# PNP-team/ZPrize23-gpu-submission

Hardware: AMD Instinct MI355X
Metric: gen_proof wall-clock (s), HEIGHT=15 Poseidon tree, 1/2/4/8 MI355X + HBM GB/s (lower is better)
Workload: dtype u64

## Files before the change

include/pnp_plonk.h:

```cpp
#ifndef PNP_PLONK_H
#define PNP_PLONK_H

#include <stdint.h>
#include <stddef.h>

#ifdef __cplusplus
extern "C" {
#endif


typedef struct {
    uint64_t a_eval[4];
    uint64_t b_eval[4];
    uint64_t c_eval[4];
    uint64_t d_eval[4];
} WireEvaluationsC;

typedef struct {
    uint64_t left_sigma_eval[4];
    uint64_t right_sigma_eval[4];
    uint64_t out_sigma_eval[4];
    uint64_t permutation_eval[4];
} PermutationEvaluationsC;

// ... 194 lines not shown
#define PNP_EX_TAG_STATUS    0x57A7A500ULL
#define PNP_EX_TAG_DEVICE    0xDE71CE00ULL
typedef int (*pnp_alltoall_fn)(void *user, uint64_t bytes_per_peer);
typedef int (*pnp_alltoallv_fn)(void *user, const uint64_t *send_bytes, const uint64_t *recv_bytes);
int pnp_ctx_stream(pnp_ctx *ctx, void **stream);
int pnp_set_exchange_ordered(pnp_ctx *ctx, int ordered);
int pnp_set_msm_shard(pnp_ctx *ctx, int rank, int world, pnp_allgather_fn allgather,
                      void *user, uint64_t *d_xbuf, uint64_t xbuf_bytes);
int pnp_set_exchange_a2a(pnp_ctx *ctx, pnp_alltoall_fn alltoall, void *user, uint64_t *d_a2a,
                         uint64_t a2a_bytes);
int pnp_set_exchange_v(pnp_ctx *ctx, pnp_alltoallv_fn alltoallv, void *user, uint64_t *d_send,
                       uint64_t *d_recv, uint64_t capacity_bytes);


int pnp_sync(pnp_ctx *ctx);

int pnp_ntt(pnp_ctx *ctx, uint64_t *d_inout, uint32_t lg_n, int inverse, int coset);

int pnp_coset_lde8(pnp_ctx *ctx, const uint64_t *d_coeffs, uint64_t *d_out8, uint32_t lg_n);

int pnp_commit(pnp_ctx *ctx, const uint64_t *d_points, const uint64_t *d_scalars,
               uint64_t n, CommitmentC *out);

int pnp_commit_ck(pnp_ctx *ctx, const uint64_t *d_scalars, uint64_t n, CommitmentC *out);

int pnp_commit_evals(pnp_ctx *ctx, const uint64_t *d_evals, uint64_t n, CommitmentC *out);

int pnp_hbm_usage(pnp_ctx *ctx, uint64_t out[6]);

int pnp_commit_segments(pnp_ctx *ctx, const uint64_t *d_points, uint64_t n_points, int B,
                        const uint64_t *seg_off, const uint64_t *const *d_scalars, uint64_t n,
                        CommitmentC *out);

int pnp_wire_sigma(pnp_ctx *ctx, const uint32_t *const d_var[4], uint64_t n_gates, uint64_t n_vars,
                   uint32_t lg_n, uint32_t *d_next, uint64_t *const d_sigma[4]);

int pnp_gather_witness(pnp_ctx *ctx, const uint32_t *const d_var[4], uint64_t n_gates,
                       const uint64_t *d_values, uint64_t n_vars, uint32_t lg_n, uint64_t *const d_w[4]);

int pnp_poly_eval(pnp_ctx *ctx, const uint64_t *d_coeffs, uint64_t n,
                  const uint64_t x[4], uint64_t out[4]);

int pnp_poly_div_linear(pnp_ctx *ctx, uint64_t *d_poly, uint64_t n, const uint64_t z[4]);

int pnp_prefix_product(pnp_ctx *ctx, uint64_t *d_inout, uint64_t n);

int pnp_batch_inverse(pnp_ctx *ctx, uint64_t *d_inout, uint64_t n);


int pnp_synth_random_fr(pnp_ctx *ctx, uint64_t *d_out, uint64_t n, uint64_t seed);
int pnp_synth_srs(pnp_ctx *ctx, uint64_t *d_out, uint64_t n, const uint64_t tau[4]);
int pnp_synth_circuit(pnp_ctx *ctx, uint64_t *const w[4], uint64_t *const sel[9],
                      uint64_t *const sigma[4], uint64_t n, uint64_t n_gates, uint64_t pi_pos,
                      const uint64_t pi_canon[4]);
int pnp_synth_merkle(pnp_ctx *ctx, uint32_t height, const uint64_t *consts, const uint64_t *d_leaves,
                     const uint64_t *d_blind, uint64_t *d_nodes, uint64_t *const w[4], uint64_t *const sel[9],
                     uint64_t *const sigma[4], uint64_t n, uint64_t root_canon[4]);
int pnp_synth_coset_consts(pnp_ctx *ctx, uint64_t *d_vh, uint64_t *d_x, uint32_t lg_n);

#ifdef __cplusplus
}
#endif

#ifdef __cplusplus
static_assert(sizeof(CommitmentC) == 96, "CommitmentC layout (lib.rs:231-235)");
static_assert(sizeof(ProofEvaluationsC) == 26 * 32, "ProofEvaluationsC layout");
// ... 13 lines not shown
```

zprize23-gpu-submission_amd/csrc/abi.cpp:

```cpp
#include <algorithm>
#include <dlfcn.h>
#include <array>
#include <atomic>
#include <chrono>
#include <mutex>
#include <set>
#include <thread>
#include <stdarg.h>
#include <stdlib.h>
#include <string.h>
#include "context.h"
#include "ec.cuh"
#include "protocol.h"

namespace pnp {

static thread_local char g_err[512] = "";

void set_error(const char *fmt, ...) {
    va_list ap;
    va_start(ap, fmt);
    vsnprintf(g_err, sizeof g_err, fmt, ap);
    va_end(ap);
}
// ... 767 lines not shown
}

int pnp_commit_segments(pnp_ctx *ctx, const uint64_t *d_points, uint64_t n_points, int B, const uint64_t *seg_off,
                        const uint64_t *const *d_scalars, uint64_t n, CommitmentC *out) {
    if (!ctx || !out || !seg_off || !d_scalars || B < 1 || B > 16 || (n_points && !d_points)) return PNP_E_ARG;
    for (int b = 0; b < B; b++) {
        if ((n && !d_scalars[b]) || seg_off[b] > n_points || n > n_points - seg_off[b]) {
            set_error("commit segments: MSM %d covers points [%llu, %llu) of %llu", b,
                      (unsigned long long)seg_off[b], (unsigned long long)(seg_off[b] + n),
                      (unsigned long long)n_points);
            return PNP_E_ARG;
        }
    }
    if (ctx->msm.world > 1) {
        set_error("commit segments: single-GPU operator");
        return PNP_E_ARG;
    }
    PNP_TRY({
        std::vector<uint64_t> xyzz((size_t)B * 24), aff((size_t)B * 12);
        if (n != 0) {
            DevBuf tab;
            msm_build_table(tab, d_points, n_points, msm_fold_c(n, ctx->msm.fold_c), ctx->stream);
            MsmSegs segs;
            segs.n_table = n_points;
            for (int b = 0; b < B; b++) segs.off[b] = seg_off[b];
            segs.c = msm_fold_c(n, ctx->msm.fold_c);
            msm_run_batch(ctx->msm, nullptr, d_scalars, B, n, xyzz.data(), ctx->stream, tab.u64(), false, &segs);
        }
        xyzz_to_affine_batch_host(xyzz.data(), B, aff.data());
        for (int b = 0; b < B; b++) {
            memcpy(out[b].x, &aff[12 * b], 48);
            memcpy(out[b].y, &aff[12 * b + 6], 48);
        }
    });
}

int pnp_poly_eval(pnp_ctx *ctx, const uint64_t *d, uint64_t n, const uint64_t x[4], uint64_t out[4]) {
    if (!ctx || !d || !x || !out) return PNP_E_ARG;
    PNP_TRY({
        Fr r;
        k_poly_eval(d, n, from_u64_limbs<FrP>(x), ctx->scratch_a, &r, ctx->stream);
        to_u64_limbs(r, out);
    });
}

int pnp_poly_div_linear(pnp_ctx *ctx, uint64_t *d, uint64_t n, const uint64_t z[4]) {
    if (!ctx || !d || !z) return PNP_E_ARG;
    PNP_TRY(k_poly_div_linear(d, n, from_u64_limbs<FrP>(z), ctx->scratch_a, ctx->stream));
}

int pnp_prefix_product(pnp_ctx *ctx, uint64_t *d, uint64_t n) {
    if (!ctx || !d) return PNP_E_ARG;
    PNP_TRY(k_prefix_product(d, n, ctx->scratch_a, ctx->stream));
}

int pnp_batch_inverse(pnp_ctx *ctx, uint64_t *d, uint64_t n) {
    if (!ctx || !d) return PNP_E_ARG;
    PNP_TRY(k_batch_inverse(d, n, ctx->scratch_a, ctx->stream));
}

int pnp_synth_random_fr(pnp_ctx *ctx, uint64_t *d, uint64_t n, uint64_t seed) {
    if (!ctx || !d) return PNP_E_ARG;
    PNP_TRY(k_random_fr(d, n, seed, ctx->stream));
}

int pnp_synth_srs(pnp_ctx *ctx, uint64_t *d, uint64_t n, const uint64_t tau[4]) {
// ... 615 lines not shown
                if (p && !pnp::k_any_nonzero(p, 4 * D, ctx->scratch_b, ctx->stream)) p = nullptr;
                if (p && kPkKinds[f] == kTable) {
                    pnp::DevBuf &t = tabc[f - kTableField[0]];
                    t.alloc(32 * D);
                    PNP_HIP(hipMemcpyAsync(t.p, p, 32 * D, hipMemcpyDeviceToDevice, ctx->stream));
                    pnp::ntt_run(ctx->ntt, t.u64(), lg, true, false, ctx->stream);
                    p = t.u64();
                }
                if (!p) {
                    memset(vk->polys[k].x, 0, 48);
                    memcpy(vk->polys[k].y, one, 48);
                    continue;
                }
                sc.push_back(p);
                oc.push_back(&vk->polys[k]);
            }
            for (size_t b = 0; b < sc.size(); b += 8)
                pnp::commit_affine_batch(ctx, sc.data() + b, (int)std::min<size_t>(8, sc.size() - b), D, oc.data() + b);
            lap(t_vk);
        }
        ctx->stages.push_back({"pre_upload", t_up});
        ctx->stages.push_back({"pre_permutation", t_perm});
        ctx->stages.push_back({"pre_intt", t_intt});
        ctx->stages.push_back({"pre_derive", t_derive});
        ctx->stages.push_back({"pre_vk", t_vk});
        ctx->stages.push_back({"pre_h2d_bytes", h2d_bytes});
    });
}

}

namespace {

void adopt_ck(pnp_ctx *ctx, pnp::DevBuf &up, uint64_t n_points) {
    const bool same = ctx->ck_owned.p && ctx->ck_dev == ctx->ck_owned.u64() && ctx->ck_points == n_points &&
                      !pnp::k_any_diff(up.u64(), ctx->ck_owned.u64(), 12 * n_points, ctx->scratch_b, ctx->stream);
    PNP_HIP(hipStreamSynchronize(ctx->stream));
    if (!same) {
        std::swap(ctx->ck_owned, up);
        ctx->ck_dev = ctx->ck_owned.u64();
        pnp::ck_derived_reset(ctx);
    }
    ctx->ck_points = n_points;
    ctx->ck_loaded = true;
    ctx->hbm_checked = false;
}

}

extern "C" {

int pnp_load_commit_key(pnp_ctx *ctx, const CommitKeyC *ck, uint64_t n_points, int device_ptrs) {
    if (!ctx || !ck || !ck->powers_of_g || n_points == 0) return PNP_E_ARG;
    PNP_TRY({
        tables_wait(ctx);
        PNP_HIP(hipSetDevice(ctx->device));
        ctx->ck_loaded = false;
        if (device_ptrs) {
            uint64_t h[2];
            pnp::k_hash_words(ck->powers_of_g, 12 * n_points, ctx->scratch_b, ctx->stream, h);
            const bool same = ctx->ck_hash_valid && !ctx->ck_owned.p && ctx->ck_dev == ck->powers_of_g &&
                              ctx->ck_points == n_points && h[0] == ctx->ck_hash[0] && h[1] == ctx->ck_hash[1];
            ctx->ck_owned.release();
            ctx->ck_dev = ck->powers_of_g;
            ctx->ck_points = n_points;
            if (!same) pnp::ck_derived_reset(ctx);
            ctx->ck_hash[0] = h[0];
            ctx->ck_hash[1] = h[1];
            ctx->ck_hash_valid = true;
            ctx->ck_loaded = true;
            ctx->hbm_checked = false;
        } else {
            ctx->ck_hash_valid = false;
            pnp::DevBuf up(n_points * 96);
            h2d_batch(ctx, {{up.p, ck->powers_of_g, n_points * 96}});
            adopt_ck(ctx, up, n_points);
        }
    });
}

int pnp_load_commit_key_strided(pnp_ctx *ctx, const void *points, uint64_t n_points,
                                const pnp_affine_layout *layout, int device_ptrs) {
    if (!ctx || !points || !layout || n_points == 0) return PNP_E_ARG;
    const pnp_affine_layout L = *layout;
    if (L.stride % 8 || L.x_off % 8 || L.y_off % 8 || L.x_off + 48 > L.stride || L.y_off + 48 > L.stride ||
        L.inf_off >= L.stride || (L.x_off < L.y_off + 48 && L.y_off < L.x_off + 48) ||
        (L.inf_off >= L.x_off && L.inf_off < L.x_off + 48) || (L.inf_off >= L.y_off && L.inf_off < L.y_off + 48)) {
        pnp::set_error("affine layout: stride %llu, x at %llu, y at %llu, infinity at %llu is not a G1Affine layout",
                       (unsigned long long)L.stride, (unsigned long long)L.x_off, (unsigned long long)L.y_off,
                       (unsigned long long)L.inf_off);
        return PNP_E_ARG;
    }
    PNP_TRY({
        tables_wait(ctx);
        PNP_HIP(hipSetDevice(ctx->device));
        ctx->ck_loaded = false;
        pnp::DevBuf raw;
        const uint8_t *src = static_cast<const uint8_t *>(points);
        if (!device_ptrs) {
// ... 544 lines not shown
```

zprize23-gpu-submission_amd/csrc/context.h:

```cpp
#pragma once
#include "pnp_internal.h"
#include <array>
#include <atomic>
#include <memory>
#include <thread>

struct pnp_ctx {
    int device = 0;
    hipStream_t stream = nullptr;
    hipStream_t stream_lo = nullptr;
    hipEvent_t ev_fork = nullptr, ev_w8 = nullptr, ev_z8 = nullptr;
    hipStream_t side_stream();
    pnp::NttTables ntt;
    pnp::MsmWork msm;
    pnp::DevBuf scratch_a, scratch_b;
    static constexpr int kStgThreads = 6;
    void *stg_buf[2 * kStgThreads] = {};
    hipStream_t stg_st[kStgThreads] = {};
    hipEvent_t stg_ev[2 * kStgThreads] = {};

    bool pk_loaded = false;
    uint64_t pk_n = 0;
    std::vector<pnp::DevBuf> pk_owned;
    ProverKeyC pk_dev{};
    bool pk_qm_zero = false, pk_qlookup_zero = false;
    bool pk_custom_nz[4] = {};
    pnp::DevBuf pk_sigma_n[4];
    pnp::DevBuf pk_tmp[4];
    std::map<std::string, pnp::DevBuf> pk_blk;
    int pk_mb0 = 0, pk_nb = 8, pk_blk_rank = 0, pk_blk_world = 1;
    bool pk_std_coset = false;
    pnp::DevBuf pk_pinv;
    uint64_t pk_pinv_pos = ~0ULL;
    const uint64_t *blk(const char *name) const {
        auto it = pk_blk.find(name);
        return it == pk_blk.end() ? nullptr : it->second.u64();
    }
    std::map<std::string, pnp::DevBuf> pk_blk29;
    bool pk_q29 = false;
    const uint64_t *blk29(const char *name) const {
        auto it = pk_blk29.find(name);
        return it == pk_blk29.end() ? nullptr : it->second.u64();
    }
    bool wm_loaded = false;
    uint64_t wm_gates = 0, wm_vars = 0;
    pnp::DevBuf wm_var;
    pnp::DevBuf wm_qlk;
    void wire_map_drop() {
        wm_loaded = false;
        wm_gates = wm_vars = 0;
        wm_var.release();
        wm_qlk.release();
    }
    bool ck_loaded = false;
    uint64_t ck_points = 0;
    pnp::DevBuf ck_owned;
    const uint64_t *ck_dev = nullptr;
    uint64_t ck_hash[2] = {0, 0};
    bool ck_hash_valid = false;
    pnp::DevBuf ck_table;
    uint64_t ck_table_n = 0, ck_table_p0 = 0, ck_table_p1 = 0;
    pnp::DevBuf lag_points, lag_table;
    uint64_t lag_n = 0, lag_table_n = 0, lag_table_p0 = 0, lag_table_p1 = 0;
    bool lag_ok = false;
    struct WireBases {
        bool built = false, ok = false, wires_ok = false, z_ok = false;
        bool sliced = false;
        int c = 0;
        uint64_t n = 0, total = 0, m = 0, len = 0;
        uint64_t g[5] = {}, off[5] = {};
        bool ident[5] = {};
        pnp::DevBuf grp[5], rep[5];
        pnp::DevBuf scal[5];
        pnp::DevBuf table;
        pnp::DevBuf sigma;
        pnp::DevBuf flag;
        uint64_t pk_gen = 0;
    } wb;
    uint64_t pk_gen = 0;
    std::atomic<bool> hbm_lag_off{false}, hbm_groups_off{false};
    bool hbm_checked = false;
    int defer_tables = -1;
    bool defer_now = false;
    bool tables_wanted = false;
    uint64_t proofs_started = 0;
    std::thread bg;
    std::atomic<int> bg_state{0};
    std::atomic<bool> bg_cancel{false};
    hipStream_t bg_stream = nullptr;

// ... 59 lines not shown
```

zprize23-gpu-submission_amd/csrc/msm.hip:

```cpp
#include <algorithm>
#include "msm_internal.h"
#include "ec.cuh"
#include "ec29.cuh"

namespace pnp {

constexpr uint32_t KEY_ZERO = 0xFFFFFFFFu;
template <int C, class E>
__device__ __forceinline__ void digits_of(const Fr &s, int c_rt, int W_rt, int top_sh, E emit) {
    const int c = C > 0 ? C : c_rt;
    const int W = C > 0 ? (255 + C) / C : W_rt;
    const uint32_t NB = 1u << (c - 1);
    uint32_t carry = 0;
    auto digit = [&](int w) {
        const int bit = w * c;
        const int li = bit >> 5, sh = bit & 31;
        uint32_t lo32 = 0, hi32 = 0;
#pragma unroll
        for (int k = 0; k < 8; k++) {
            lo32 = li == k ? s.v[k] : lo32;
            hi32 = li + 1 == k ? s.v[k] : hi32;
        }
        const uint64_t word = lo32 | ((uint64_t)hi32 << 32);
        uint32_t raw = (uint32_t)(word >> sh) & ((1u << c) - 1);
// ... 28 lines not shown
        digits_of<20>(s, c, W, top_sh, emit);
    else
        digits_of<0>(s, c, W, top_sh, emit);
}
__global__ void k_digits(const uint64_t *scalars, uint64_t n, int c, int W, int top_sh, uint32_t *keys) {
    uint64_t i = blockIdx.x * (uint64_t)blockDim.x + threadIdx.x;
    if (i >= n) return;
    scalar_digits(scalars, i, n, c, W, top_sh, keys, [](uint32_t) {});
}

constexpr int MSM_BATCH_MAX = 16;
struct KeyRows {
    uint64_t n;
    int vstride, off, rows;
    uint32_t id_row0;
    uint64_t id_mul;
    uint64_t id_base = 0;
    int nseg = 0;
    uint64_t seg_off[MSM_BATCH_MAX] = {};
};

#ifndef PNP_SORT_CB
#define PNP_SORT_CB 9
#endif
constexpr int SORT_CB = PNP_SORT_CB;
constexpr int SORT_FB_MAX = 11;
static_assert(SORT_CB >= 1 && SORT_CB <= 12, "PNP_SORT_CB out of range (LDS budget of k_coarse_scatter)");
__device__ __forceinline__ uint64_t cidx(int v, int nv, uint32_t b, int NBc, int wmaj, int ch, int nch) {
    if (wmaj <= 1) return ((uint64_t)v * NBc + b) * nch + ch;
    const uint32_t nbl = (uint32_t)NBc / wmaj;
    return (((uint64_t)(b / nbl) * nv + v) * nbl + b % nbl) * nch + ch;
}

__global__ __launch_bounds__(1024) void k_coarse_hist(const uint32_t *keys, KeyRows kr, int fb,
                                                      int NBc, uint64_t chunk, int nch,
                                                      uint32_t *counts, int wmaj = 1) {
    __shared__ uint32_t hist[1 << SORT_CB];
    const int v = blockIdx.y, ch = blockIdx.x;
    for (int b = threadIdx.x; b < NBc; b += blockDim.x) hist[b] = 0;
    __syncthreads();
    const uint64_t n = kr.n;
    uint64_t lo = (uint64_t)ch * chunk, hi = lo + chunk < n ? lo + chunk : n;
    const uint32_t *kb = keys + ((uint64_t)v * kr.vstride + kr.off) * n;
    const bool vec = ((n | chunk) & 3) == 0;
    for (int r = 0; r < kr.rows; r++) {
        const uint32_t *k = kb + (uint64_t)r * n;
        if (vec) {
            for (uint64_t i = lo + 4 * threadIdx.x; i < hi; i += 4 * blockDim.x) {
                uint4 q = *reinterpret_cast<const uint4 *>(k + i);
                uint32_t w[4] = {q.x, q.y, q.z, q.w};
#pragma unroll
                for (int j = 0; j < 4; j++)
                    if (w[j] != KEY_ZERO) atomicAdd(&hist[(w[j] & 0x7FFFFFFFu) >> fb], 1u);
            }
        } else {
            for (uint64_t i = lo + threadIdx.x; i < hi; i += blockDim.x) {
                uint32_t key = k[i];
                if (key != KEY_ZERO) atomicAdd(&hist[(key & 0x7FFFFFFFu) >> fb], 1u);
            }
        }
    }
    __syncthreads();
    for (int b = threadIdx.x; b < NBc; b += blockDim.x) counts[cidx(v, gridDim.y, b, NBc, wmaj, ch, nch)] = hist[b];
}

struct ScalarPtrs {
    static constexpr int MAX = MSM_BATCH_MAX;
    const uint64_t *p[MAX];
};
__global__ __launch_bounds__(1024) void k_digits_hist(ScalarPtrs sp, uint64_t n, int c, int W, int top_sh, int fb,
                                                      int NBc,
                                                      uint64_t chunk, int nch, uint32_t *keys, uint32_t *counts,
                                                      int wmaj = 1) {
    __shared__ uint32_t hist[1 << SORT_CB];
    const int v = blockIdx.y, ch = blockIdx.x;
    for (int b = threadIdx.x; b < NBc; b += blockDim.x) hist[b] = 0;
    __syncthreads();
    const uint64_t lo = (uint64_t)ch * chunk, hi = lo + chunk < n ? lo + chunk : n;
    uint32_t *kv = keys + (uint64_t)v * W * n;
    for (uint64_t i = lo + threadIdx.x; i < hi; i += blockDim.x)
        scalar_digits(sp.p[v], i, n, c, W, top_sh, kv, [&](uint32_t key) {
            if (key != KEY_ZERO) atomicAdd(&hist[(key & 0x7FFFFFFFu) >> fb], 1u);
        });
    __syncthreads();
    for (int b = threadIdx.x; b < NBc; b += blockDim.x) counts[cidx(v, gridDim.y, b, NBc, wmaj, ch, nch)] = hist[b];
}

__global__ __launch_bounds__(256) void k_scan_tiles(uint32_t *d, uint64_t n, uint32_t *tile_sums) {
    __shared__ uint32_t wsum[4];
    uint64_t base = (uint64_t)blockIdx.x * 1024;
    uint32_t v[4], loc = 0;
    for (int k = 0; k < 4; k++) {
        uint64_t i = base + threadIdx.x * 4 + k;
        v[k] = i < n ? d[i] : 0;
        loc += v[k];
    }
    uint32_t x = loc;
    int lane = threadIdx.x & 63, wv = threadIdx.x >> 6;
    for (int off = 1; off < 64; off <<= 1) {
        uint32_t y = __shfl_up(x, off, 64);
        if (lane >= off) x += y;
    }
    if (lane == 63) wsum[wv] = x;
    __syncthreads();
    uint32_t wpre = 0;
    for (int j = 0; j < wv; j++) wpre += wsum[j];
    uint32_t excl = wpre + x - loc;
    for (int k = 0; k < 4; k++) {
        uint64_t i = base + threadIdx.x * 4 + k;
        if (i < n) d[i] = excl;
        excl += v[k];
    }
    if (threadIdx.x == 255) tile_sums[blockIdx.x] = wpre + x;
}
__global__ void k_scan_add(uint32_t *d, uint64_t n, const uint32_t *tile_pre) {
    uint64_t i = blockIdx.x * (uint64_t)blockDim.x + threadIdx.x;
    if (i < n) d[i] += tile_pre[i >> 10];
}
// ... 292 lines not shown
    __syncthreads();
    const uint32_t a = std::min((ps + 3) & ~3u, pe), b = std::max(pe & ~3u, a);
    {
        const uint32_t step = 4 * blockDim.x;
        uint32_t k = a + 4 * threadIdx.x;
        for (; k + 3 * step < b; k += 4 * step) {
            uint2 q[4];
#pragma unroll
            for (int u = 0; u < 4; u++) q[u] = *reinterpret_cast<const uint2 *>(fk + k + u * step);
#pragma unroll
            for (int u = 0; u < 4; u++) {
                atomicAdd(&h[q[u].x & 0xFFFF], 1u);
                atomicAdd(&h[q[u].x >> 16], 1u);
                atomicAdd(&h[q[u].y & 0xFFFF], 1u);
                atomicAdd(&h[q[u].y >> 16], 1u);
            }
        }
        for (; k < b; k += step) {
            const uint2 q = *reinterpret_cast<const uint2 *>(fk + k);
            atomicAdd(&h[q.x & 0xFFFF], 1u);
            atomicAdd(&h[q.x >> 16], 1u);
            atomicAdd(&h[q.y & 0xFFFF], 1u);
            atomicAdd(&h[q.y >> 16], 1u);
        }
    }
    for (uint32_t k = ps + threadIdx.x; k < a; k += blockDim.x) atomicAdd(&h[fk[k]], 1u);
    for (uint32_t k = b + threadIdx.x; k < pe; k += blockDim.x) atomicAdd(&h[fk[k]], 1u);
    __syncthreads();
    tile_scan(h, lofs, NF, wsum);
    __syncthreads();
    for (int f = threadIdx.x; f < NF; f += blockDim.x) h[f] = ps + lofs[f];
    __syncthreads();
    for (int f = threadIdx.x; f < NF; f += blockDim.x) bstart[p * NF + f] = h[f];
    constexpr int PER = TILE_F / 1024;
    uint32_t ne[PER], nf[PER];
    auto load_tile = [&](uint32_t tb) {
#pragma unroll
        for (int j = 0; j < PER; j++) {
            uint32_t k = tb + threadIdx.x + j * 1024;
            nf[j] = 0;
            ne[j] = 0xFFFFFFFFu;
            if (k < pe) {
                nf[j] = fk[k];
                ne[j] = ent[k];
            }
        }
    };
    if (ps < pe) load_tile(ps);
    for (uint32_t tb = ps; tb < pe; tb += TILE_F) {
        uint32_t e[PER], rank[PER];
        uint32_t f[PER];
#pragma unroll
        for (int j = 0; j < PER; j++) e[j] = ne[j], f[j] = nf[j];
#if PNP_SORT_PREFETCH
        if (pe - tb > (uint32_t)TILE_F) load_tile(tb + TILE_F);
#endif
#pragma unroll
        for (int j = 0; j < PER; j++)
            if (tb + threadIdx.x + j * 1024 < pe) rank[j] = atomicAdd(&lh[f[j]], 1u);
        __syncthreads();
        tile_scan(lh, lofs, NF, wsum);
        __syncthreads();
#pragma unroll
        for (int j = 0; j < PER; j++) {
            uint32_t k = tb + threadIdx.x + j * 1024;
            if (k < pe) {
// ... 286 lines not shown
static constexpr uint64_t PT29 = PNP_PT29;

#ifndef PNP_ACC_GLDS
#define PNP_ACC_GLDS 1
#endif
typedef __attribute__((address_space(3))) void lds_void_t;
typedef __attribute__((address_space(1))) void glob_void_t;
__device__ __forceinline__ void stage_point(const uint32_t *p, uint4 *st) {
#pragma unroll
    for (int c = 0; c < 7; c++)
        __builtin_amdgcn_global_load_lds((glob_void_t *)(p + 4 * c), (lds_void_t *)(st + 64 * c), 16, 0, 0);
}
__device__ __forceinline__ void unstage_point(const uint4 *st, F29 &x, F29 &y) {
    uint32_t w[28];
#pragma unroll
    for (int c = 0; c < 7; c++) {
        const uint4 v = st[64 * c];
        w[4 * c] = v.x;
        w[4 * c + 1] = v.y;
        w[4 * c + 2] = v.z;
        w[4 * c + 3] = v.w;
    }
#pragma unroll
    for (int i = 0; i < 14; i++) {
        x.l[i] = w[i];
        y.l[i] = w[14 + i];
    }
}

__global__ __launch_bounds__(256, PNP_ACC_WAVES) void k_accumulate29(const uint32_t *pts29, const uint32_t *sorted,
                                                      const uint32_t *offs, uint64_t U, uint64_t nthr, uint32_t S,
                                                      uint32_t *buckets, uint32_t *head,
                                                      uint32_t *tail, uint32_t *tailb, uint32_t *redo,
                                                      uint32_t *nredo, uint32_t *tlist) {
#if PNP_ACC_GLDS == 1
    __shared__ uint4 stage[4 * 7 * 64];
    __shared__ uint32_t sidx[4 * 64];
    const uint32_t wv = threadIdx.x >> 6, ln = threadIdx.x & 63;
    uint4 *wave_base = stage + 7 * 64 * wv;
    uint32_t *idx_base = sidx + 64 * wv;
#endif
    uint64_t t = blockIdx.x * (uint64_t)blockDim.x + threadIdx.x;
    const uint32_t total = offs[U];
    S = acc_seg(offs, U, nthr, S);
    const uint64_t lo64 = t * S;
    if (lo64 >= total) return;
    const uint32_t lo = (uint32_t)lo64;
    const uint32_t hi = lo + S < total ? lo + S : total;
    uint64_t a = 0, b = U;
    while (b - a > 1) {
        uint64_t m = (a + b) >> 1;
        if (offs[m] <= lo) a = m; else b = m;
    }
    uint64_t cur = a;
    bool first = offs[cur] < lo;
    uint32_t next = offs[cur + 1];
    bool ok = true, fresh = true;
    Xyzz29 acc;
#if PNP_ACC_GLDS == 1
    uint32_t e = sorted[lo];
    stage_point(pts29 + PT29 * (e & 0x7FFFFFFFu), wave_base);
    if (lo + 1 < hi)
        __builtin_amdgcn_global_load_lds((glob_void_t *)(sorted + lo + 1), (lds_void_t *)idx_base, 4, 0, 0);
#elif PNP_ACC_GLDS == 2
    uint32_t e = sorted[lo];
    F29 nx = load29(pts29 + PT29 * (e & 0x7FFFFFFFu)), ny = load29(pts29 + PT29 * (e & 0x7FFFFFFFu) + 14);
    uint32_t en = lo + 1 < hi ? sorted[lo + 1] : 0u;
#endif
    for (uint32_t k = lo; k < hi; k++) {
        if (k == next) {
            ok &= store29(first ? head + 56 * t : buckets + 56 * cur, acc);
            first = false;
            fresh = true;
            cur = next_bucket(offs, 1, U, cur + 1, k, next);
        }
#if PNP_ACC_GLDS == 2
        F29 x = nx, y = ny;
        const uint32_t ecur = e;
        if (k + 1 < hi) {
            const uint32_t *p = pts29 + PT29 * (en & 0x7FFFFFFFu);
            nx = load29(p);
            ny = load29(p + 14);
            e = en;
            if (k + 2 < hi) en = sorted[k + 2];
        }
        if (ecur >> 31) y = neg29(y, F29_KA);
#elif PNP_ACC_GLDS
        F29 x, y;
        __builtin_amdgcn_s_waitcnt(0x0F70);
        unstage_point(wave_base + ln, x, y);
        const uint32_t en = idx_base[ln];
        __builtin_amdgcn_s_waitcnt(0xC07F);
        const uint32_t ecur = e;
        if (k + 1 < hi) {
            stage_point(pts29 + PT29 * (en & 0x7FFFFFFFu), wave_base);
            if (k + 2 < hi)
                __builtin_amdgcn_global_load_lds((glob_void_t *)(sorted + k + 2), (lds_void_t *)idx_base, 4, 0,
                                                 0);
            e = en;
        }
        if (ecur >> 31) y = neg29(y, F29_KA);
#else
        const uint32_t e = sorted[k];
        const uint32_t *p = pts29 + PT29 * (e & 0x7FFFFFFFu);
        F29 x = load29(p), y = load29(p + 14);
        if (e >> 31) y = neg29(y, F29_KA);
#endif
        if (fresh) {
            acc.x = x;
            acc.y = y;
            acc.zz = acc.zzz = const29(F29_ONE);
            fresh = false;
        } else {
            madd29(acc, x, y);
        }
    }
    const bool to_tail = !first && next > hi;
    ok &= store29(first ? head + 56 * t : (to_tail ? tail + 56 * t : buckets + 56 * cur), acc);
    tailb[t] = to_tail ? (uint32_t)cur : NO_TAIL;
    const uint64_t m = __ballot(to_tail);
    if (to_tail) {
        const int leader = __ffsll((unsigned long long)m) - 1;
        const uint32_t below = __builtin_amdgcn_mbcnt_hi((uint32_t)(m >> 32), __builtin_amdgcn_mbcnt_lo((uint32_t)m, 0u));
        uint32_t base = 0;
        if (below == 0) base = atomicAdd(tlist, (uint32_t)__popcll(m));
        base = __shfl(base, leader);
        tlist[1 + base + below] = (uint32_t)t;
    }
    if (!ok) redo[atomicAdd(nredo, 1u)] = (uint32_t)t;
}

constexpr int WCTR_SLOTS = 64;
__global__ __launch_bounds__(1024) void k_count_pieces(const uint32_t *offs, uint64_t WB, uint64_t nthr, uint32_t S,
                                                       unsigned long long *ctr) {
    S = acc_seg(offs, WB, nthr, S);
    __shared__ uint32_t part[16];
    const uint64_t b = blockIdx.x * (uint64_t)blockDim.x + threadIdx.x;
    bool fresh = false;
    if (b < WB) {
        const uint32_t o = offs[b];
        fresh = offs[b + 1] > o && (o % S) != 0;
    }
    const unsigned long long m = __ballot(fresh);
    if ((threadIdx.x & 63) == 0) part[threadIdx.x >> 6] = (uint32_t)__popcll(m);
    __syncthreads();
    if (threadIdx.x == 0) {
        uint32_t t = 0;
        for (int w = 0; w < (int)(blockDim.x >> 6); w++) t += part[w];
        if (t) atomicAdd(&ctr[1 + (blockIdx.x & (WCTR_SLOTS - 1))], (unsigned long long)t);
        if (blockIdx.x == 0) {
            const unsigned long long tot = offs[WB];
            ctr[0] = tot;
            atomicAdd(&ctr[1], (tot + S - 1) / S);
        }
    }
}

__global__ __launch_bounds__(64) void k_accumulate_redo(const uint32_t *pts29, const uint32_t *sorted,
                                                        const uint32_t *offs, uint64_t U, uint64_t nthr, uint32_t S,
                                                        uint32_t *buckets, uint32_t *head,
                                                        uint32_t *tail, const uint32_t *redo,
                                                        const uint32_t *nredo) {
    auto ld = [pts29](uint32_t i, Fq &x, Fq &y) {
        x = to_fq32(load29(pts29 + PT29 * i));
        y = to_fq32(load29(pts29 + PT29 * i + 14));
// ... 107 lines not shown
    PNP_HIP(hipStreamSynchronize(s));
}

void xyzz_to_affine_dev(const uint64_t *xyzz, uint64_t n, uint64_t *aff, hipStream_t s) {
    const uint32_t CH = 64;
    const uint64_t lanes = (n + CH - 1) / CH;
    DevBuf pre(n * 48);
    hipLaunchKernelGGL(k_table_affine, dim3((uint32_t)((lanes + 255) / 256)), dim3(256), 0, s, xyzz, n, CH,
                       pre.u64(), aff);
    PNP_HIP(hipGetLastError());
    PNP_HIP(hipStreamSynchronize(s));
}

static void put_xyzz(const Xyzz &r, uint64_t *o) {
    to_u64_limbs(r.x, o);
    to_u64_limbs(r.y, o + 6);
    to_u64_limbs(r.zz, o + 12);
    to_u64_limbs(r.zzz, o + 18);
}
static Xyzz get_xyzz(const uint64_t *e) {
    Xyzz p;
    p.x = from_u64_limbs<FqP>(e);
    p.y = from_u64_limbs<FqP>(e + 6);
    p.zz = from_u64_limbs<FqP>(e + 12);
    p.zzz = from_u64_limbs<FqP>(e + 18);
    return p;
}

struct GroupPlan {
    KeyRows kr;
    int nv;
};

static void sort_group(MsmWork &wk, MsmGroup &gb, const uint32_t *keys, const GroupPlan &gp,
                       const MsmCfg &g, hipStream_t s, const uint64_t *const *scalars = nullptr) {
    const int nv = gp.nv;
    const uint64_t n = gp.kr.n, WB = (uint64_t)nv * g.NB;
    const int nch0 = std::max(1, 512 / std::max(nv, 1));
    const uint64_t chunk = std::max<uint64_t>(1024, (n + nch0 - 1) / nch0);
    const int nch = (int)((n + chunk - 1) / chunk);
    const int cb = std::min(SORT_CB, g.c - 1), fb = g.c - 1 - cb, NBc = 1 << cb;
    if (fb > SORT_FB_MAX) {
        set_error("msm: window of %d bits exceeds the sort's %d", g.c, SORT_CB + SORT_FB_MAX + 1);
        throw Error(PNP_E_ARG);
    }
    const uint64_t nbins = (uint64_t)nv * NBc;
    const uint64_t nent = (uint64_t)nv * gp.kr.rows * n;
    auto need = [](DevBuf &b, size_t bytes) { if (b.bytes < bytes) b.alloc(bytes); };
    need(gb.counts, (nbins * nch + 1) * 4);
    need(gb.offsets, (WB + 1) * 4);
    need(gb.ent, nent * 4 + 4);
    need(gb.fkey, nent * 2 + 8);
    need(gb.sorted, nent * 4 + 4);
    uint32_t *counts = static_cast<uint32_t *>(gb.counts.p);
    uint32_t *bstart = static_cast<uint32_t *>(gb.offsets.p);
    dim3 grid((uint32_t)nch, (uint32_t)nv);
    if (scalars) {
        ScalarPtrs sp{};
        for (int v = 0; v < nv; v++) sp.p[v] = scalars[v];
        hipLaunchKernelGGL(k_digits_hist, grid, dim3(1024), 0, s, sp, n, g.c, g.W, g.top_sh, fb, NBc, chunk, nch,
                           const_cast<uint32_t *>(keys), counts, 1);
    } else {
        hipLaunchKernelGGL(k_coarse_hist, grid, dim3(1024), 0, s, keys, gp.kr, fb, NBc, chunk, nch, counts);
    }
    PNP_HIP(hipGetLastError());
    const uint64_t ncount = nbins * nch;
    PNP_HIP(hipMemsetAsync(counts + ncount, 0, 4, s));
    scan_u32(counts, ncount + 1, gb.scan_tmp, s);
    uint32_t *ent = static_cast<uint32_t *>(gb.ent.p);
    uint16_t *fk = static_cast<uint16_t *>(gb.fkey.p);
    hipLaunchKernelGGL(k_coarse_scatter, grid, dim3(1024), 0, s, keys, gp.kr, fb, NBc, chunk, nch,
                       counts, ent, fk);
    PNP_HIP(hipGetLastError());
    hipLaunchKernelGGL(k_fine_sort, dim3((uint32_t)nbins), dim3(1024), 0, s, ent, fk, counts, nch, fb,
                       bstart, static_cast<uint32_t *>(gb.sorted.p));
    PNP_HIP(hipGetLastError());
    PNP_HIP(hipMemcpyAsync(bstart + WB, counts + ncount, 4, hipMemcpyDeviceToDevice, s));
}

static uint32_t acc_segment(uint64_t nent, bool folded) {
    uint32_t S = (uint32_t)std::max<uint64_t>(64, (nent >> 20) & ~7ULL);
    if (!folded) return S;
    static uint64_t slots = 0;
    if (!slots) {
        int dev = 0, cus = 0;
        PNP_HIP(hipGetDevice(&dev));
        PNP_HIP(hipDeviceGetAttribute(&cus, hipDeviceAttributeMultiprocessorCount, dev));
        slots = (uint64_t)cus * 4 * PNP_ACC_WAVES * 64;
    }
    const uint64_t per = (nent + slots - 1) / slots;
    static const uint64_t max_rounds = [] {
        const char *e = getenv("PNP_ACC_ROUNDS");
        return e && atoi(e) > 0 ? (uint64_t)atoi(e) : ~0ULL;
    }();
    const uint64_t rounds = std::min(max_rounds, std::max<uint64_t>(1, per / S));
    return (uint32_t)std::max<uint64_t>(16, (per + rounds - 1) / rounds);
}

static void accumulate_group(MsmWork &wk, MsmGroup &gb, const GroupPlan &gp, const MsmCfg &g,
                             const uint64_t *pts, const uint64_t *table, hipStream_t s, uint64_t nent = 0,
                             double alg_bytes = 0) {
    const int nv = gp.nv;
    const uint64_t n = gp.kr.n, WB = (uint64_t)nv * g.NB;
    if (!nent) nent = (uint64_t)nv * gp.kr.rows * n;
    if (alg_bytes == 0) alg_bytes = (double)n * 128.0 * nv * gp.kr.rows / g.W;
    auto need = [](DevBuf &b, size_t bytes) { if (b.bytes < bytes) b.alloc(bytes); };
    need(gb.buckets, (WB * 24 + WB * 72 + 64) * 8);
    const uint32_t *bstart = static_cast<const uint32_t *>(gb.offsets.p);
    const uint32_t *sorted = static_cast<const uint32_t *>(gb.sorted.p);
    uint64_t *bk = gb.buckets.u64();
    hipEvent_t ev0 = nullptr;
    if (wk.timer) wk.timer->begin("msm_accumulate", s, ev0);
    const uint32_t S = acc_segment(nent, table != nullptr);
    const uint64_t nthr = (nent + S - 1) / S;
    if (table) {
        need(gb.seg, (WB + 2 * nthr) * 224 + nthr * 4 + (nthr + 1) * 4);
        uint32_t *bk29 = static_cast<uint32_t *>(gb.seg.p);
        uint32_t *head = bk29 + 56 * WB, *tail = head + 56 * nthr, *tailb = tail + 56 * nthr;
        uint32_t *tlist = tailb + nthr;
        PNP_HIP(hipMemsetAsync(tlist, 0, 4, s));
        need(gb.redo, nthr * 4 + 16);
        uint32_t *nredo = static_cast<uint32_t *>(gb.redo.p), *redo = nredo + 4;
        PNP_HIP(hipMemsetAsync(nredo, 0, 4, s));
        const uint32_t *t29 = reinterpret_cast<const uint32_t *>(table);
        const uint32_t blocks = (uint32_t)((nthr + 255) / 256);
        hipLaunchKernelGGL(k_accumulate29, dim3(blocks), dim3(256), 0, s, t29, sorted, bstart, WB, nthr, S, bk29,
                           head, tail, tailb, redo, nredo, tlist);
        PNP_HIP(hipGetLastError());
        hipLaunchKernelGGL(k_accumulate_redo, dim3((uint32_t)std::min<uint64_t>((nthr + 63) / 64, 1024)), dim3(64), 0, s, t29,
                           sorted, bstart, WB, nthr, S, bk29, head, tail, redo, nredo);
        PNP_HIP(hipGetLastError());
        need(gb.exc, 16);
        PNP_HIP(hipMemsetAsync(gb.exc.p, 0, 4, s));
        gb.S = S;
        gb.pieces = (uint32_t)(nent / WB / S + 1);
        gb.nthr = nthr;
        need(gb.heavy, (WB + 1) * 4);
        msm_merge_pieces29(bstart, WB, S, nthr, tailb, tlist, bk29, head, tail, static_cast<uint32_t *>(gb.exc.p),
                           static_cast<uint32_t *>(gb.heavy.p), s);
    } else {
        need(gb.seg, nthr * 2 * 24 * 8);
        uint64_t *head = gb.seg.u64(), *tail = head + nthr * 24;
        hipLaunchKernelGGL(k_accumulate_flat, dim3((uint32_t)((nthr + 255) / 256)), dim3(256), 0, s, pts,
                           sorted, bstart, 1, WB, S, bk, head, tail);
        PNP_HIP(hipGetLastError());
        msm_merge_pieces(bstart, 1, WB, S, (uint32_t)(nent / WB / S + 1), head, tail, bk, s);
    }
    if (wk.timer) {
        wk.timer->end("msm_accumulate", s, ev0, alg_bytes);
        wk.timer->credit("msm_entries_dense", (double)nent);
        if (table) {
            need(gb.wctr, 8 * (1 + WCTR_SLOTS));
            PNP_HIP(hipMemsetAsync(gb.wctr.p, 0, 8 * (1 + WCTR_SLOTS), s));
            hipLaunchKernelGGL(k_count_pieces, dim3((uint32_t)((WB + 1023) / 1024)), dim3(1024), 0, s, bstart, WB, nthr, S,
                               static_cast<unsigned long long *>(gb.wctr.p));
            PNP_HIP(hipGetLastError());
            gb.wctr_live = true;
        }
    }
}

static void wctr_fetch(MsmGroup &gb, hipStream_t s) {
    if (gb.wctr_live) PNP_HIP(hipMemcpyAsync(gb.wctr_h, gb.wctr.p, 8 * (1 + WCTR_SLOTS), hipMemcpyDeviceToHost, s));
}
static void wctr_credit(MsmWork &wk, MsmGroup &gb) {
    if (!gb.wctr_live) return;
    gb.wctr_live = false;
    if (!wk.timer) return;
    unsigned long long pieces = 0;
    for (int k = 1; k <= WCTR_SLOTS; k++) pieces += gb.wctr_h[k];
    wk.timer->credit("msm_entries", (double)gb.wctr_h[0]);
    wk.timer->credit("msm_madds", (double)(gb.wctr_h[0] - pieces));
}

static const uint64_t *reduce_group(MsmGroup &gb, const GroupPlan &gp, const MsmCfg &g, hipStream_t s,
                                    bool folded) {
    const uint64_t WB = (uint64_t)gp.nv * g.NB;
    uint64_t *bk = gb.buckets.u64();
    if (folded)
        return msm_reduce29(static_cast<const uint32_t *>(gb.seg.p), static_cast<const uint32_t *>(gb.offsets.p),
                            (uint64_t)gp.nv, g.NB,
                            reinterpret_cast<uint32_t *>(bk), static_cast<uint32_t *>(gb.exc.p), s);
    return msm_reduce(bk, (uint64_t)gp.nv, g.NB, bk + WB * 24, s);
}

static const uint64_t *reduce_group_exact(MsmGroup &gb, const GroupPlan &gp, const MsmCfg &g, hipStream_t s) {
    const uint64_t WB = (uint64_t)gp.nv * g.NB;
    uint64_t *bk = gb.buckets.u64();
    const uint32_t *bk29 = static_cast<const uint32_t *>(gb.seg.p);
    const uint32_t *head = bk29 + 56 * WB, *tail = head + 56 * gb.nthr;
    msm_merge_pieces29_exact(static_cast<const uint32_t *>(gb.offsets.p), WB, gb.S, gb.nthr, gb.pieces, bk29, head, tail,
                             bk, s);
    return msm_reduce(bk, (uint64_t)gp.nv, g.NB, bk + WB * 24, s);
}

static hipEvent_t ev_get(MsmWork &wk, int i) {
    if (!wk.ev[i]) PNP_HIP(hipEventCreateWithFlags(&wk.ev[i], hipEventDisableTiming));
    return wk.ev[i];
}

static int pipe_min_b() {
    static const int v = [] {
        const char *e = getenv("PNP_MSM_PIPE");
        return e ? std::max(1, atoi(e)) : 0;
    }();
    return v;
}
static bool pipe_off() { return pipe_min_b() == 0; }

static void msm_local_batch(MsmWork &wk, const uint64_t *d_points, const uint64_t *const *d_scalars,
                            int B, uint64_t n, uint64_t *h_xyzz, hipStream_t s,
                            const uint64_t *table, uint64_t n_table = 0, uint64_t id_base = 0,
                            const uint64_t *seg_off = nullptr, int cfg_c = 0) {
    if (n == 0 || B == 0) {
        for (int b = 0; b < B; b++) put_xyzz(Xyzz::inf(), h_xyzz + 24 * b);
// ... 29 lines not shown
        kr.vstride = g.W, kr.off = 0, kr.rows = g.W, kr.id_row0 = 0, kr.id_mul = n_table;
        kr.id_base = id_base;
        gp[0] = {kr, B};
    } else if (B >= 2) {
        const int h = (B + 1) / 2;
        kr.vstride = g.W, kr.off = 0, kr.rows = g.W, kr.id_row0 = 0, kr.id_mul = n_table, kr.id_base = id_base;
        gp[0] = {kr, h};
        kr.off = h * g.W;
        gp[1] = {kr, B - h};
        first[1] = h;
        ng = 2;
    } else if (g.W >= 2) {
        const int h = g.W / 2;
        kr.vstride = g.W, kr.off = 0, kr.rows = h, kr.id_row0 = 0, kr.id_mul = n_table, kr.id_base = id_base;
        gp[0] = {kr, 1};
        kr.off = h, kr.rows = g.W - h, kr.id_row0 = h;
        gp[1] = {kr, 1};
        ng = 2;
    } else {
        kr.vstride = g.W, kr.off = 0, kr.rows = g.W, kr.id_row0 = 0, kr.id_mul = n_table, kr.id_base = id_base;
        gp[0] = {kr, 1};
    }
    if (seg_off) {
        for (int k = 0; k < ng; k++) {
            gp[k].kr.nseg = gp[k].nv;
            for (int v = 0; v < gp[k].nv; v++) gp[k].kr.seg_off[v] = seg_off[B == 1 ? 0 : first[k] + v];
        }
    }
    const uint64_t *pts = folded ? table : d_points;
    const uint64_t *res[2] = {nullptr, nullptr};
    if (ng == 1) {
        sort_group(wk, wk.grp[0], keys, gp[0], g, s, fuse ? d_scalars : nullptr);
        accumulate_group(wk, wk.grp[0], gp[0], g, pts, table, s);
        res[0] = reduce_group(wk.grp[0], gp[0], g, s, folded);
    } else {
        if (!wk.s2) PNP_HIP(hipStreamCreateWithFlags(&wk.s2, hipStreamNonBlocking));
        hipEvent_t evD = ev_get(wk, 0), evS1 = ev_get(wk, 1), evA0 = ev_get(wk, 2), evR0 = ev_get(wk, 3);
        PNP_HIP(hipEventRecord(evD, s));
        PNP_HIP(hipStreamWaitEvent(wk.s2, evD, 0));
        sort_group(wk, wk.grp[1], keys, gp[1], g, wk.s2);
        PNP_HIP(hipEventRecord(evS1, wk.s2));
        sort_group(wk, wk.grp[0], keys, gp[0], g, s);
        accumulate_group(wk, wk.grp[0], gp[0], g, pts, table, s);
        PNP_HIP(hipEventRecord(evA0, s));
        PNP_HIP(hipStreamWaitEvent(wk.s2, evA0, 0));
        res[0] = reduce_group(wk.grp[0], gp[0], g, wk.s2, folded);
        PNP_HIP(hipEventRecord(evR0, wk.s2));
        PNP_HIP(hipStreamWaitEvent(s, evS1, 0));
        accumulate_group(wk, wk.grp[1], gp[1], g, pts, table, s);
        res[1] = reduce_group(wk.grp[1], gp[1], g, s, folded);
        PNP_HIP(hipStreamWaitEvent(s, evR0, 0));
    }
    std::vector<uint64_t> win[2];
    uint32_t exc[2] = {0, 0}, nredo[2] = {0, 0};
    for (int k = 0; k < ng; k++) {
        win[k].resize((size_t)gp[k].nv * 24);
        PNP_HIP(hipMemcpyAsync(win[k].data(), res[k], win[k].size() * 8, hipMemcpyDeviceToHost, s));
        if (folded) {
            PNP_HIP(hipMemcpyAsync(&exc[k], wk.grp[k].exc.p, 4, hipMemcpyDeviceToHost, s));
            PNP_HIP(hipMemcpyAsync(&nredo[k], wk.grp[k].redo.p, 4, hipMemcpyDeviceToHost, s));
            wctr_fetch(wk.grp[k], s);
        }
    }
    PNP_HIP(hipStreamSynchronize(s));
    for (int k = 0; k < ng; k++) wctr_credit(wk, wk.grp[k]);
    if (wk.timer) wk.timer->credit("msm_redo_lanes", (double)nredo[0] + nredo[1]);
    for (int k = 0; k < ng; k++) {
        if (!exc[k]) continue;
        if (wk.timer) wk.timer->credit("msm_exact_fallback", 1);
        res[k] = reduce_group_exact(wk.grp[k], gp[k], g, s);
        PNP_HIP(hipMemcpyAsync(win[k].data(), res[k], win[k].size() * 8, hipMemcpyDeviceToHost, s));
        PNP_HIP(hipStreamSynchronize(s));
    }
    if (wk.timer) wk.timer->collect();
    for (int b = 0; b < B; b++) put_xyzz(Xyzz::inf(), h_xyzz + 24 * b);
    for (int k = 0; k < ng; k++) {
        for (int v = 0; v < gp[k].nv; v++) {
            if (folded) {
                const int b = B == 1 ? 0 : first[k] + v;
                put_xyzz(add(get_xyzz(h_xyzz + 24 * b), get_xyzz(&win[k][(size_t)v * 24])), h_xyzz + 24 * b);
            }
        }
    }
    if (!folded) {
        for (int b = 0; b < B; b++) {
            Xyzz acc = Xyzz::inf();
            for (int w = g.W - 1; w >= 0; w--) {
                for (int k = 0; k < g.c; k++) acc = dbl(acc);
                acc = add(acc, get_xyzz(&win[0][((size_t)b * g.W + w) * 24]));
            }
            put_xyzz(acc, h_xyzz + 24 * b);
        }
    }
}

std::vector<uint64_t> rank_allgather(MsmWork &wk, hipStream_t s, const uint64_t *mine, int k, uint64_t tag) {
    const int W = wk.world;
    const uint64_t words = (uint64_t)k + 1, slot = 8 * words;
// ... 109 lines not shown
        const uint64_t nruns = 2 * per_d * W;
        need(wk.slot_dev, (nruns + per_d + 1 + 2 + W) * 4);
        uint32_t *rt = static_cast<uint32_t *>(wk.slot_dev.p), *o0 = rt + nruns, *flags = o0 + per_d + 1,
                 *dcnt = flags + 2;
        hipLaunchKernelGGL(k_slot_header, dim3((uint32_t)W), dim3(256), 0, s, counts, (uint32_t)per_d, nch, W,
                           (uint32_t)slot_recs, (uint32_t)cap, wk.v_send, dcnt);
        PNP_HIP(hipGetLastError());
        if (n) {
            hipLaunchKernelGGL(k_coarse_scatter, grid, dim3(1024), 0, s, keys, kr, fb, NBc, chunk, nch, counts,
                               nullptr, nullptr, W, wk.v_send, (uint32_t)slot_recs, hdr, (uint32_t)cap);
            PNP_HIP(hipGetLastError());
        }
        ex_fence(wk, s);
        std::vector<uint64_t> eq(W, slot_recs * 8);
        if (int rc = wk.alltoallv(wk.v_user, eq.data(), eq.data())) {
            set_error("msm bucket shard: slot all-to-all failed (%d)", rc);
            throw Error(PNP_E_DEVICE);
        }
        need(gb.offsets, (WB + 1) * 4);
        need(gb.sorted, W * cap * 4 + 4);
        uint32_t *bstart = static_cast<uint32_t *>(gb.offsets.p);
        hipLaunchKernelGGL(k_slot_runs, dim3(1), dim3(1024), 0, s, wk.v_recv, W, (uint32_t)slot_recs, hdr,
                           (uint32_t)per_d, (uint32_t)cap, reinterpret_cast<uint2 *>(rt), o0, bstart + WB, flags);
        PNP_HIP(hipGetLastError());
        hipLaunchKernelGGL(k_fine_sort_runs, dim3((uint32_t)per_d), dim3(1024), 0, s, wk.v_recv,
                           reinterpret_cast<const uint2 *>(rt), W, o0, fb, bstart,
                           static_cast<uint32_t *>(gb.sorted.p));
        PNP_HIP(hipGetLastError());
        MsmCfg gl = g;
        gl.NB = (int)NBloc;
        GroupPlan gp;
        gp.kr = kr;
        gp.nv = B;
        accumulate_group(wk, gb, gp, gl, nullptr, table, s, W * cap, (double)W * cap * 128.0 / g.W);
        const uint64_t *res = reduce_group(gb, gp, gl, s, true);
        std::vector<uint64_t> ts((size_t)B * 48);
        uint32_t exc = 0, nredo = 0, fl[2] = {0, 0};
        std::vector<uint32_t> dc(W);
        PNP_HIP(hipMemcpyAsync(ts.data(), res, ts.size() * 8, hipMemcpyDeviceToHost, s));
        PNP_HIP(hipMemcpyAsync(&exc, gb.exc.p, 4, hipMemcpyDeviceToHost, s));
        PNP_HIP(hipMemcpyAsync(&nredo, gb.redo.p, 4, hipMemcpyDeviceToHost, s));
        PNP_HIP(hipMemcpyAsync(fl, flags, 8, hipMemcpyDeviceToHost, s));
        PNP_HIP(hipMemcpyAsync(dc.data(), dcnt, 4 * W, hipMemcpyDeviceToHost, s));
        wctr_fetch(gb, s);
        PNP_HIP(hipStreamSynchronize(s));
        wk.slot_runs++;
        if (fl[0]) {
            gb.wctr_live = false;
            wk.slot_overflows++;
            if (wk.timer) {
                wk.timer->credit("msm_slot_overflows", 1);
                wk.timer->collect();
            }
        } else {
            wctr_credit(wk, gb);
            if (wk.timer) {
                wk.timer->credit("msm_slot_batches", 1);
                wk.timer->credit("msm_redo_lanes", (double)nredo);
                uint64_t mx = 0, sum = 0;
                for (uint32_t c : dc) mx = std::max<uint64_t>(mx, c), sum += c;
                wk.timer->credit("msm_dest_max", (double)mx);
                wk.timer->credit("msm_dest_sum", (double)sum);
            }
            if (exc) {
                if (wk.timer) wk.timer->credit("msm_exact_fallback", 1);
                res = reduce_group_exact(gb, gp, gl, s);
                PNP_HIP(hipMemcpyAsync(ts.data(), res, ts.size() * 8, hipMemcpyDeviceToHost, s));
                PNP_HIP(hipStreamSynchronize(s));
            }
            if (wk.timer) wk.timer->collect();
            for (int b = 0; b < B; b++) {
                const Xyzz T = get_xyzz(&ts[24 * (size_t)b]), S = get_xyzz(&ts[24 * ((size_t)B + b)]);
                put_xyzz(lo_w ? add(T, mul_small(S, lo_w)) : T, part + 24 * (size_t)b);
            }
            return true;
        }
    }
    std::vector<uint32_t> offs(ncount + 1);
// ... 72 lines not shown
                set_error("msm bucket shard: rank %d sent %llu records, its bin counts say %llu", r,
                          (unsigned long long)(recv_b[r] / 8), (unsigned long long)(at - base));
                throw Error(PNP_E_DEVICE);
            }
            base = at;
        }
        uint64_t o = 0;
        for (uint64_t p = 0; p < per_d; p++) {
            out0[p] = (uint32_t)o;
            for (int r = 0; r < W; r++) o += runs[2 * (p * W + r) + 1];
        }
        out0[per_d] = (uint32_t)o;
    }
    const uint64_t R = out0[per_d];
    need(gb.offsets, (WB + 1) * 4);
    need(gb.sorted, R * 4 + 4);
    need(gb.ent, (runs.size() + out0.size()) * 4);
    uint32_t *bstart = static_cast<uint32_t *>(gb.offsets.p);
    uint32_t *rt = static_cast<uint32_t *>(gb.ent.p), *o0 = rt + runs.size();
    PNP_HIP(hipMemcpyAsync(rt, runs.data(), runs.size() * 4, hipMemcpyHostToDevice, s));
    PNP_HIP(hipMemcpyAsync(o0, out0.data(), out0.size() * 4, hipMemcpyHostToDevice, s));
    hipLaunchKernelGGL(k_fine_sort_runs, dim3((uint32_t)per_d), dim3(1024), 0, s, wk.v_recv,
                       reinterpret_cast<const uint2 *>(rt), W, o0, fb, bstart, static_cast<uint32_t *>(gb.sorted.p));
    PNP_HIP(hipGetLastError());
    PNP_HIP(hipMemcpyAsync(bstart + WB, o0 + per_d, 4, hipMemcpyDeviceToDevice, s));
    MsmCfg gl = g;
    gl.NB = (int)NBloc;
    GroupPlan gp;
    gp.kr = kr;
    gp.nv = B;
    std::vector<uint64_t> ts((size_t)B * 48);
    for (int b = 0; b < 2 * B; b++) put_xyzz(Xyzz::inf(), &ts[24 * (size_t)b]);
    if (R) {
        accumulate_group(wk, gb, gp, gl, nullptr, table, s, R, (double)R * 128.0 / g.W);
        const uint64_t *res = reduce_group(gb, gp, gl, s, true);
        uint32_t exc = 0, nredo = 0;
        PNP_HIP(hipMemcpyAsync(ts.data(), res, ts.size() * 8, hipMemcpyDeviceToHost, s));
        PNP_HIP(hipMemcpyAsync(&exc, gb.exc.p, 4, hipMemcpyDeviceToHost, s));
        PNP_HIP(hipMemcpyAsync(&nredo, gb.redo.p, 4, hipMemcpyDeviceToHost, s));
        wctr_fetch(gb, s);
        PNP_HIP(hipStreamSynchronize(s));
        wctr_credit(wk, gb);
        if (wk.timer) wk.timer->credit("msm_redo_lanes", (double)nredo);
        if (exc) {
            if (wk.timer) wk.timer->credit("msm_exact_fallback", 1);
            res = reduce_group_exact(gb, gp, gl, s);
            PNP_HIP(hipMemcpyAsync(ts.data(), res, ts.size() * 8, hipMemcpyDeviceToHost, s));
            PNP_HIP(hipStreamSynchronize(s));
        }
        if (wk.timer) wk.timer->collect();
    }
    for (int b = 0; b < B; b++) {
        const Xyzz T = get_xyzz(&ts[24 * (size_t)b]), S = get_xyzz(&ts[24 * ((size_t)B + b)]);
        put_xyzz(lo_w ? add(T, mul_small(S, lo_w)) : T, part + 24 * (size_t)b);
    }
    return true;
}

int msm_fold_c(uint64_t n_points, int fold_c) { return msm_cfg(n_points, fold_c, true).c; }

uint64_t msm_table_bytes(uint64_t n_points, uint64_t n_cfg, int fold_c) {
    return (uint64_t)msm_cfg(n_cfg, fold_c, true).W * n_points * PT29 * 4;
}
uint64_t msm_table_build_bytes(uint64_t n_points) { return n_points * (96 + 96 + 192 + 48); }
uint64_t msm_work_bytes(uint64_t n_pts, uint64_t n_cfg, int fold_c, int B, uint64_t v_bytes, int world) {
    const MsmCfg g = msm_cfg(n_cfg, fold_c, true);
    const bool buckets = world > 1 && v_bytes > 0;
    const uint64_t WB = (uint64_t)B * (buckets ? g.NB / world : g.NB);
    const uint64_t nent = (uint64_t)B * g.W * n_pts;
    const uint64_t digits = nent * 4, counts = (uint64_t)B * 512 * 1024 * 4 + (WB + 1) * 4;
    const uint64_t acc_ent = buckets ? v_bytes / 8 : nent;
    const uint64_t sort = buckets ? acc_ent * 4 : nent * (4 + 2 + 4);
    const uint64_t S = std::max<uint32_t>(16, acc_segment(acc_ent, true));
    const uint64_t nthr = (acc_ent + S - 1) / S;
    const uint64_t acc = (WB + 2 * nthr) * 224 + nthr * 12 + (WB + 1) * 4 + (WB * 24 + WB * 72 + 64) * 8;
    return digits + counts + sort + acc;
}
uint64_t msm_work_held(const MsmWork &wk) {
    uint64_t b = wk.digits.bytes + wk.part_counts.bytes + wk.rec_counts.bytes;
    for (const MsmGroup &g : wk.grp)
        b += g.counts.bytes + g.offsets.bytes + g.scan_tmp.bytes + g.ent.bytes + g.fkey.bytes + g.sorted.bytes +
             g.buckets.bytes + g.seg.bytes + g.redo.bytes + g.exc.bytes + g.heavy.bytes + g.wctr.bytes;
    return b;
}

void msm_point_range(uint64_t n, int rank, int world, uint64_t &p0, uint64_t &p1) {
    const uint64_t per = (n + world - 1) / world;
    p0 = std::min<uint64_t>((uint64_t)rank * per, n);
    p1 = std::min<uint64_t>(p0 + per, n);
}

void msm_run_batch(MsmWork &wk, const uint64_t *d_points, const uint64_t *const *d_scalars, int B,
                   uint64_t n, uint64_t *h_xyzz, hipStream_t s, const uint64_t *table,
                   bool scalars_local, const MsmSegs *segs) {
    if (segs && (!table || B > MSM_BATCH_MAX)) {
        set_error("msm: point segments need a folded table and at most %d MSMs", MSM_BATCH_MAX);
        throw Error(PNP_E_ARG);
    }
    if (wk.timer) wk.timer->credit("msm_scalar_bytes", 32.0 * (double)B * n / wk.world);
    if (wk.world == 1) {
        if (segs)
            msm_local_batch(wk, nullptr, d_scalars, B, n, h_xyzz, s, table, segs->n_table, 0, segs->off, segs->c);
        else
            msm_local_batch(wk, d_points, d_scalars, B, n, h_xyzz, s, table);
        return;
    }
    uint64_t p0, p1;
    msm_point_range(n, wk.rank, wk.world, p0, p1);
    std::vector<const uint64_t *> sc(B);
    for (int b = 0; b < B; b++) sc[b] = scalars_local ? d_scalars[b] : d_scalars[b] + 4 * p0;
    std::vector<uint64_t> part((size_t)B * 24);
    const bool full = table && (wk.full_table() || (segs && !segs->sliced));
    const uint64_t n_tab = segs ? segs->n_table : n;
    const uint64_t *off = segs ? segs->off : nullptr;
    if (segs && segs->sliced && wk.full_table()) {
// ... 49 lines not shown
```

zprize23-gpu-submission_amd/csrc/msm_internal.h:

```cpp
#pragma once
#include "pnp_internal.h"

namespace pnp {

struct MsmCfg {
    int c, W, NB;
    int top_sh;
};

inline MsmCfg msm_cfg(uint64_t n, int c = 0, bool folded = false) {
    MsmCfg g;
    int lg = 0;
    while ((1ULL << lg) < n) lg++;
    if (folded)
        g.c = lg >= 19 ? 20 : (lg - 3 < 4 ? 4 : lg - 3);
    else
        g.c = lg >= 20 ? 16 : (lg - 3 < 4 ? 4 : lg - 3);
    if (c > 0) g.c = c;
    g.W = (256 + g.c - 1) / g.c;
    g.NB = 1 << (g.c - 1);
    const int top_bits = 255 - g.c * (g.W - 1);
    g.top_sh = folded && top_bits >= 0 && g.c - 1 - top_bits > 0 ? g.c - 1 - top_bits : 0;
    return g;
}

void msm_merge_pieces(const uint32_t *offs, int nch, uint64_t U, uint32_t S, uint32_t pieces,
                      const uint64_t *head, const uint64_t *tail, uint64_t *bk, hipStream_t s);

constexpr uint32_t NO_TAIL = 0xFFFFFFFFu;

#ifndef PNP_ACC_DEVSEG
#define PNP_ACC_DEVSEG 0
#endif
__device__ __forceinline__ uint32_t acc_seg(const uint32_t *offs, uint64_t U, uint64_t nthr, uint32_t S) {
#if PNP_ACC_DEVSEG
    const uint64_t total = offs[U];
    uint64_t d = (total + nthr - 1) / nthr;
    d = d < 16 ? 16 : d;
    return d < S ? (uint32_t)d : S;
#else
    (void)offs, (void)U, (void)nthr;
    return S;
#endif
}
void msm_merge_pieces29(const uint32_t *offs, uint64_t U, uint32_t S, uint64_t nthr, const uint32_t *tailb,
                        const uint32_t *tlist, uint32_t *bk29, const uint32_t *head, const uint32_t *tail, uint32_t *exc,
                        uint32_t *heavy, hipStream_t s);
void msm_merge_pieces29_exact(const uint32_t *offs, uint64_t U, uint32_t S, uint64_t nthr, uint32_t pieces,
                              const uint32_t *bk29, const uint32_t *head, const uint32_t *tail, uint64_t *bk,
                              hipStream_t s);


const uint64_t *msm_reduce(const uint64_t *bk, uint64_t nwin, int NB, uint64_t *scratch,
                           hipStream_t s);
const uint64_t *msm_reduce29(const uint32_t *bk29, const uint32_t *offs, uint64_t nwin, int NB,
                             uint32_t *scratch, uint32_t *exc, hipStream_t s);

}
```

zprize23-gpu-submission_amd/csrc/msm_reduce.hip:

```cpp
#include "msm_internal.h"
#include "ec.cuh"
#include "ec29.cuh"

namespace pnp {

__global__ __launch_bounds__(256) void k_tree_leaf(const uint64_t *bk, uint64_t nout, uint64_t *out) {
    uint64_t t = blockIdx.x * (uint64_t)blockDim.x + threadIdx.x;
    if (t >= nout) return;
    Xyzz b1 = load_xyzz(bk + 24 * (2 * t + 1));
    Xyzz S = add(load_xyzz(bk + 24 * (2 * t)), b1);
    uint64_t *o = out + 72 * t;
    store_xyzz(o, S);
    store_xyzz(o + 24, add(S, b1));
    store_xyzz(o + 48, dbl(S));
}

#ifndef PNP_LEAF_W
#define PNP_LEAF_W 8
#endif
template <int LW>
__global__ __launch_bounds__(256) void k_tree_leafw(const uint64_t *bk, uint64_t nout, uint64_t *out) {
    uint64_t t = blockIdx.x * (uint64_t)blockDim.x + threadIdx.x;
    if (t >= nout) return;
    const uint64_t *b = bk + 24 * LW * t;
// ... 45 lines not shown
            if (t0 != t1) {
                live = true;
#pragma unroll 1
                for (uint32_t k = j; k <= t1 - t0; k += G)
                    acc = add(acc, load_xyzz(k == 0 ? tail + 24ULL * t0 : head + 24ULL * (t0 + k)));
            }
        }
    }
    uint64_t *mine = lds + 24 * threadIdx.x;
    for (int h = G / 2; h >= 1; h /= 2) {
        store_xyzz(mine, acc);
        __syncthreads();
        if (live && j < h) acc = add(acc, load_xyzz(mine + 24 * h));
        __syncthreads();
    }
    if (live && j == 0) store_xyzz(bk + 24 * g, acc);
}

void msm_merge_pieces(const uint32_t *offs, int nch, uint64_t U, uint32_t S, uint32_t pieces,
                      const uint64_t *head, const uint64_t *tail, uint64_t *bk, hipStream_t s) {
    int G = 1;
    while (G < 8 && (uint32_t)G * 8 <= pieces) G *= 2;
    const uint64_t blocks = (U * G + 255) / 256;
    hipLaunchKernelGGL(k_merge_pieces, dim3((uint32_t)blocks), dim3(256), 0, s, offs, nch, U, S, G,
                       head, tail, bk);
    PNP_HIP(hipGetLastError());
}

#ifndef PNP_MERGE_HEAVY
#define PNP_MERGE_HEAVY 16
#endif
constexpr uint32_t MERGE_HEAVY = PNP_MERGE_HEAVY;
__global__ __launch_bounds__(256) void k_merge_tails29(const uint32_t *offs, uint64_t U, uint64_t nthr, uint32_t S,
                                                       const uint32_t *tailb, const uint32_t *tlist, uint32_t *bk29,
                                                       const uint32_t *head, const uint32_t *tail, uint32_t *exc,
                                                       uint32_t *heavy, uint32_t *nheavy) {
    const uint64_t q = blockIdx.x * (uint64_t)blockDim.x + threadIdx.x;
    if (q >= tlist[0]) return;
    S = acc_seg(offs, U, nthr, S);
    const uint64_t t = tlist[1 + q];
    const uint32_t u = tailb[t];
    const uint32_t t1 = (offs[u + 1] - 1) / S;
    if (t1 - (uint32_t)t >= MERGE_HEAVY) {
        heavy[atomicAdd(nheavy, 1u)] = u;
        return;
    }
    Xyzz29 acc = load_xyzz29(tail + 56 * t);
#pragma unroll 1
    for (uint32_t k = (uint32_t)t + 1; k <= t1; k++) acc = xadd29_inf(acc, load_xyzz29(head + 56ULL * k), exc);
    store_xyzz29(bk29 + 56ULL * u, acc);
}

__global__ __launch_bounds__(256) void k_merge_heavy29(const uint32_t *offs, uint64_t U, uint64_t nthr, uint32_t S,
                                                       uint32_t *bk29, const uint32_t *head, const uint32_t *tail,
                                                       uint32_t *exc, const uint32_t *heavy, const uint32_t *nheavy) {
    __shared__ uint32_t lds[256 * 56];
    const uint32_t cnt = *nheavy;
    S = acc_seg(offs, U, nthr, S);
    uint32_t *mine = lds + 56 * threadIdx.x;
    for (uint32_t q = blockIdx.x; q < cnt; q += gridDim.x) {
        const uint32_t g = heavy[q];
        const uint32_t t0 = offs[g] / S, t1 = (offs[g + 1] - 1) / S;
        Xyzz29 acc = inf29();
#pragma unroll 1
        for (uint32_t k = threadIdx.x; k <= t1 - t0; k += blockDim.x)
            acc = xadd29_inf(acc, load_xyzz29(k == 0 ? tail + 56ULL * t0 : head + 56ULL * (t0 + k)), exc);
        uint32_t h0 = 1;
        while (2 * h0 < t1 - t0 + 1 && 2 * h0 < blockDim.x) h0 *= 2;
        for (uint32_t h = h0; h >= 1; h /= 2) {
            store_xyzz29(mine, acc);
            __syncthreads();
            if (threadIdx.x < h) acc = xadd29_inf(acc, load_xyzz29(mine + 56 * h), exc);
            __syncthreads();
        }
        if (threadIdx.x == 0) store_xyzz29(bk29 + 56ULL * g, acc);
        __syncthreads();
    }
}

void msm_merge_pieces29(const uint32_t *offs, uint64_t U, uint32_t S, uint64_t nthr, const uint32_t *tailb,
                        const uint32_t *tlist, uint32_t *bk29, const uint32_t *head, const uint32_t *tail,
                        uint32_t *exc, uint32_t *heavy, hipStream_t s) {
    uint32_t *nheavy = heavy, *list = heavy + 1;
    PNP_HIP(hipMemsetAsync(nheavy, 0, 4, s));
    hipLaunchKernelGGL(k_merge_tails29, dim3((uint32_t)((nthr + 255) / 256)), dim3(256), 0, s, offs, U, nthr, S,
                       tailb, tlist, bk29, head, tail, exc, list, nheavy);
    PNP_HIP(hipGetLastError());
    hipLaunchKernelGGL(k_merge_heavy29, dim3(256), dim3(256), 0, s, offs, U, nthr, S, bk29, head, tail, exc, list,
                       nheavy);
    PNP_HIP(hipGetLastError());
}

__device__ __forceinline__ Xyzz piece29(const uint32_t *p) { return to32(load_xyzz29(p)); }
__global__ __launch_bounds__(256) void k_merge_pieces29_exact(const uint32_t *offs, uint64_t U, uint64_t nthr,
                                                              uint32_t S, int G, const uint32_t *bk29,
                                                              const uint32_t *head, const uint32_t *tail,
                                                              uint64_t *bk) {
    __shared__ uint64_t lds[256 * 24];
    S = acc_seg(offs, U, nthr, S);
    const uint64_t g = (blockIdx.x * (uint64_t)blockDim.x + threadIdx.x) / G;
    const int j = threadIdx.x % G;
    bool live = false;
    Xyzz acc = Xyzz::inf();
    if (g < U) {
        uint32_t s0 = offs[g], e0 = offs[g + 1];
        if (s0 != e0) {
            live = true;
            uint32_t t0 = s0 / S, t1 = (e0 - 1) / S;
            if (t0 == t1) {
                if (j == 0) acc = piece29(bk29 + 56 * g);
            } else {
#pragma unroll 1
                for (uint32_t k = j; k <= t1 - t0; k += G)
                    acc = add(acc, piece29(k == 0 ? tail + 56ULL * t0 : head + 56ULL * (t0 + k)));
            }
        } else if (j == 0) {
            store_xyzz(bk + 24 * g, Xyzz::inf());
        }
    }
    uint64_t *mine = lds + 24 * threadIdx.x;
    for (int h = G / 2; h >= 1; h /= 2) {
// ... 172 lines not shown
            tis = tis && zero29(T.zz);
        } else {
            S = xadd29w_inf(S, load_xyzz29(bk + 56 * (u0 + k)), r, exc);
            const bool tinf = zero29(T.zz);
            T = xadd29w_inf(T, S, r, exc);
            tis = tinf;
        }
    }
    uint32_t *o = out + 168 * t;
    store_f29(o + 14 * r, qsel(r, S.x, S.y, S.zz, S.zzz));
    store_f29(o + 56 + 14 * r, qsel(r, T.x, T.y, T.zz, T.zzz));
    Xyzz29 D = S;
#pragma unroll 1
    for (int k = 1; k < LW; k *= 2) D = xdbl29w_inf(D, r);
    store_f29(o + 112 + 14 * r, qsel(r, D.x, D.y, D.zz, D.zzz));
}

__global__ void k_tree_roots29(const uint32_t *in, uint64_t n, uint64_t *out) {
    uint64_t t = blockIdx.x * (uint64_t)blockDim.x + threadIdx.x;
    if (t >= n) return;
    store_xyzz(out + 24 * t, to32(load_xyzz29(in + 168 * t + 56)));
    store_xyzz(out + 24 * (n + t), to32(load_xyzz29(in + 168 * t)));
}

__global__ void k_tree_roots29w(const uint32_t *in, uint64_t n, uint64_t *out) {
    const uint64_t t = (blockIdx.x * (uint64_t)blockDim.x + threadIdx.x) >> 2;
    if (t >= n) return;
    const int r = (int)(threadIdx.x & 3);
    store_fq(out + 24 * t + 6 * r, to_fq32(load29(in + 168 * t + 56 + 14 * r)));
    store_fq(out + 24 * (n + t) + 6 * r, to_fq32(load29(in + 168 * t + 14 * r)));
}

const uint64_t *msm_reduce29(const uint32_t *bk29, const uint32_t *offs, uint64_t nwin, int NB,
                             uint32_t *scratch, uint32_t *exc, hipStream_t s) {
#ifndef PNP_LEAF_SMALL4
#define PNP_LEAF_SMALL4 1
#endif
    const int LW = NB >= 2 * PNP_LEAF_W ? (PNP_LEAF_SMALL4 && NB <= (1 << 16) && PNP_LEAF_W > 4 ? 4 : PNP_LEAF_W) : 2;
    if (NB < 2 * LW) {
        set_error("msm_reduce29: %d buckets per window", NB);
        throw Error(PNP_E_ARG);
    }
    uint64_t m = nwin * (uint64_t)NB / LW;
    uint32_t *a = scratch, *b = scratch + 168 * m;
    uint64_t *roots = reinterpret_cast<uint64_t *>(scratch + 252 * m);
    const dim3 lgrid((uint32_t)((m + 255) / 256));
    static const uint64_t leaf_wide = [] {
        const char *e = getenv("PNP_LEAF_WIDE");
        return (uint64_t)(e ? atoll(e) : 32768);
    }();
    const dim3 wgrid((uint32_t)((4 * m + 255) / 256));
    if (LW == 4 && m <= leaf_wide)
        hipLaunchKernelGGL(k_tree_leafw29w<4>, wgrid, dim3(256), 0, s, bk29, offs, m, a, exc);
    else if (LW == 2)
        hipLaunchKernelGGL(k_tree_leafw29<2>, lgrid, dim3(256), 0, s, bk29, offs, m, a, exc);
    else if (LW == 4)
        hipLaunchKernelGGL(k_tree_leafw29<4>, lgrid, dim3(256), 0, s, bk29, offs, m, a, exc);
    else
        hipLaunchKernelGGL(k_tree_leafw29<PNP_LEAF_W>, lgrid, dim3(256), 0, s, bk29, offs, m, a, exc);
    PNP_HIP(hipGetLastError());
    static const uint64_t wide_max = [] {
        const char *e = getenv("PNP_TREE_WIDE");
        return (uint64_t)(e ? atoll(e) : 16384);
    }();
    while (m > nwin) {
        m /= 2;
        if (m <= wide_max)
            hipLaunchKernelGGL(k_tree_level29w, dim3((uint32_t)((4 * m + 255) / 256), 3), dim3(256), 0, s, a, m, b,
                               exc);
        else
            hipLaunchKernelGGL(k_tree_level29, dim3((uint32_t)((m + 255) / 256), 3), dim3(256), 0, s, a, m, b, exc);
        PNP_HIP(hipGetLastError());
        std::swap(a, b);
    }
    hipLaunchKernelGGL(k_tree_roots29w, dim3((uint32_t)((4 * nwin + 255) / 256)), dim3(256), 0, s, a, nwin, roots);
    PNP_HIP(hipGetLastError());
    return roots;
}
// ... 32 lines not shown
```

zprize23-gpu-submission_amd/csrc/pnp_internal.h:

```cpp
#pragma once
#include <hip/hip_runtime.h>
#include <stdint.h>
#include <stdio.h>
#include <map>
#include <string>
#include <tuple>
#include <vector>
#include "field.cuh"
#include "../../include/pnp_plonk.h"

namespace pnp {

void set_error(const char *fmt, ...);

#define PNP_HIP(expr)                                                              \
    do {                                                                           \
        hipError_t e_ = (expr);                                                    \
        if (e_ != hipSuccess) {                                                    \
            ::pnp::set_error("%s:%d %s: %s", __FILE__, __LINE__, #expr,            \
                             hipGetErrorString(e_));                               \
            throw ::pnp::Error(PNP_E_DEVICE);                                      \
        }                                                                          \
    } while (0)

struct Error {
    int code;
    explicit Error(int c) : code(c) {}
};

struct DevBuf {
    void *p = nullptr;
    size_t bytes = 0;
    DevBuf() = default;
    explicit DevBuf(size_t b) { alloc(b); }
// ... 33 lines not shown
void intt_blocks(NttTables &t, uint64_t *d, uint32_t lg_n, int m0, int nb, hipStream_t s);
void t_combine(NttTables &t, const uint64_t *Y, uint64_t len, uint64_t q0, uint64_t *out,
               uint32_t lg_n, unsigned *nz, hipStream_t s);
void t_combine_blocks(NttTables &t, const uint64_t *Y, int nb, uint64_t *out, uint32_t lg_n, unsigned *nz,
                      hipStream_t s);
void to_blocks(const uint64_t *in, uint64_t *out, uint32_t lg_n, int m0, int nb, hipStream_t s);

struct KernelTimer {
    bool enabled = false;
    struct Stat {
        double ms = 0, bytes = 0;
        int launches = 0;
    };
    struct Pending {
        std::string name;
        hipEvent_t e0, e1;
        double bytes;
    };
    std::map<std::string, Stat> stats;
    std::vector<Pending> pending;
    std::vector<hipEvent_t> pool;
    hipEvent_t get();
    void begin(const char *name, hipStream_t s, hipEvent_t &e0);
    void end(const char *name, hipStream_t s, hipEvent_t e0, double bytes = 0);
    void collect();
    void credit(const char *name, double units) {
        if (enabled) stats[name].bytes += units;
    }
};

extern thread_local bool t_bg_build;
void bg_step(hipStream_t s);

struct MsmGroup {
    DevBuf counts, offsets, scan_tmp, ent, fkey, sorted, buckets, seg, redo;
    DevBuf exc;
    DevBuf heavy;
    uint32_t S = 0, pieces = 0;
    uint64_t nthr = 0;
    DevBuf wctr;
    unsigned long long wctr_h[65] = {};
    bool wctr_live = false;
};
struct MsmWork {
    DevBuf digits;
    MsmGroup grp[2];
    hipStream_t s2 = nullptr;
    hipEvent_t ev[4] = {nullptr, nullptr, nullptr, nullptr};
    KernelTimer *timer = nullptr;
    int fold_c = 0;
    int rank = 0, world = 1;
    pnp_allgather_fn allgather = nullptr;
    void *user = nullptr;
    uint64_t *xbuf = nullptr;
    uint64_t xbuf_bytes = 0;
    pnp_alltoall_fn alltoall = nullptr;
    void *a2a_user = nullptr;
    uint64_t *a2a = nullptr;
    uint64_t a2a_bytes = 0;
    pnp_alltoallv_fn alltoallv = nullptr;
    void *v_user = nullptr;
    uint64_t *v_send = nullptr, *v_recv = nullptr;
    uint64_t v_bytes = 0;
    bool ordered = false;
    bool full_table() const { return world > 1 && alltoallv != nullptr; }
    DevBuf part_counts, rec_counts;
    std::map<std::tuple<uint32_t, int, uint64_t>, uint64_t> slot_cap;
    uint32_t batch_seq = 0;
    DevBuf slot_dev;
    unsigned long long slot_runs = 0, slot_overflows = 0;
};
inline void ex_fence(const MsmWork &wk, hipStream_t s) {
    if (!wk.ordered) PNP_HIP(hipStreamSynchronize(s));
}
std::vector<uint64_t> rank_allgather(MsmWork &wk, hipStream_t s, const uint64_t *mine, int k, uint64_t tag);
void msm_run(MsmWork &w, const uint64_t *d_points, const uint64_t *d_scalars_mont, uint64_t n,
             uint64_t *h_xyzz, hipStream_t s, const uint64_t *table = nullptr);
struct MsmSegs {
    uint64_t n_table = 0;
    uint64_t off[16] = {};
    bool sliced = false;
    int c = 0;
};
int msm_fold_c(uint64_t n_points, int fold_c);
void msm_run_batch(MsmWork &w, const uint64_t *d_points, const uint64_t *const *d_scalars, int B,
                   uint64_t n, uint64_t *h_xyzz, hipStream_t s, const uint64_t *table = nullptr,
                   bool scalars_local = false, const MsmSegs *segs = nullptr);
uint64_t msm_table_bytes(uint64_t n_points, uint64_t n_cfg, int fold_c);
uint64_t msm_table_build_bytes(uint64_t n_points);
uint64_t msm_work_bytes(uint64_t n_pts, uint64_t n_cfg, int fold_c, int B, uint64_t v_bytes, int world);
uint64_t msm_work_held(const MsmWork &wk);
void msm_point_range(uint64_t n, int rank, int world, uint64_t &p0, uint64_t &p1);
void msm_build_table(DevBuf &tab, const uint64_t *d_points, uint64_t n, int c, hipStream_t s);
void xyzz_to_affine_dev(const uint64_t *xyzz, uint64_t n, uint64_t *aff, hipStream_t s);
bool srs_lagrange(const uint64_t *d_aff, uint64_t n, const Fr &omega_inv, const Fr &n_inv, uint64_t *d_out,
                  hipStream_t s);
void xyzz_to_affine_host(const uint64_t *xyzz, uint64_t *aff12);
void xyzz_to_affine_batch_host(const uint64_t *xyzz, int B, uint64_t *aff12);

void k_from_mont(uint64_t *d, uint64_t n, hipStream_t s);
void k_to_mont(uint64_t *d, uint64_t n, hipStream_t s);
void k_prefix_product(uint64_t *d, uint64_t n, DevBuf &scratch, hipStream_t s);
void k_batch_inverse(uint64_t *d, uint64_t n, DevBuf &scratch, hipStream_t s);
void k_poly_eval(const uint64_t *d, uint64_t n, const Fr &x, DevBuf &scratch, Fr *out,
                 hipStream_t s);
void k_poly_eval_multi(const uint64_t *const *polys, int npolys, uint64_t n, const Fr &x,
                       DevBuf &scratch, Fr *out, hipStream_t s);
struct EvalSet {
    const uint64_t *const *polys;
    int np;
    Fr x;
    Fr *out;
};
void k_poly_eval_sets(const EvalSet *sets, int nsets, uint64_t n, DevBuf &scratch, hipStream_t s);
void k_poly_div_linear(uint64_t *d, uint64_t n, const Fr &z, DevBuf &scratch, hipStream_t s);
void k_poly_div_linear_batch(uint64_t *const *d, const Fr *z, int K, uint64_t n, DevBuf &scratch,
                             hipStream_t s);
void k_add_powers(uint64_t *d, uint64_t len, const Fr &c, const Fr &z, hipStream_t s);
void k_random_fr(uint64_t *d, uint64_t n, uint64_t seed, hipStream_t s);
void k_geometric(uint64_t *d, uint64_t n, const Fr &c0, const Fr &r, hipStream_t s);
void k_srs(uint64_t *d, uint64_t n, const Fr &tau, hipStream_t s);
void k_coset_consts(uint64_t *vh, uint64_t *x, uint32_t lg_n, hipStream_t s);
void k_coset_blocks(uint32_t lg_n, int m0, int nb, uint64_t *lin, uint64_t *lin32, uint64_t *vh_inv,
                    uint64_t *l1_den, hipStream_t s);
// ... 25 lines not shown
```

zprize23-gpu-submission_amd/csrc/protocol.h:

```cpp
#pragma once
#include "pnp_internal.h"

namespace pnp {

__host__ __device__ inline Fr from_u64_limbs_dev(const uint64_t *l) {
    Fr r;
#pragma unroll
    for (int i = 0; i < 4; i++) {
        r.v[2 * i] = (uint32_t)l[i];
        r.v[2 * i + 1] = (uint32_t)(l[i] >> 32);
    }
    return r;
}

struct PermArgs {
    const uint64_t *w[4];
    const uint64_t *sigma[4];
    Fr bk[4];
    Fr beta, gamma, omega;
    const uint64_t *tw;
};

struct QuotArgs {
    const uint64_t *w8[4], *z8, *pi8, *f8, *t8, *h18, *h28, *z28, *l18;
// ... 14 lines not shown
    const uint64_t *vh_inv, *l1v, *pinv;
    uint32_t c_pi[9], alpha[9], alpha2[9], beta[9], gamma[9], one[9];
    uint64_t n;
    uint32_t lg_n;
};
void fr_to_r29_limbs(const Fr &a, uint32_t l[9]);
void k_quotient29(const Quot29Args &q, uint64_t N8, uint64_t *out, hipStream_t s);
void k_to_form29(const uint64_t *in, uint64_t *out, uint64_t n, hipStream_t s);

struct WidgetArgs {
    const uint64_t *w8[4], *q_l, *q_r, *q_c, *vh_inv;
    const uint64_t *sel[4];
    Fr sep[4];
    uint64_t n;
    uint32_t lg_n;
};

constexpr int LIN_MAX = 32;
struct LinArgs {
    int k;
    const uint64_t *p[LIN_MAX];
    Fr s[LIN_MAX];
};

void k_compress4(uint64_t *out, const uint64_t *t0, const uint64_t *t1, const uint64_t *t2,
                 const uint64_t *t3, const Fr &z, uint64_t n, hipStream_t s);
void k_query_f(uint64_t *out, const uint64_t *ql, uint64_t n_gates, const uint64_t *const w[4],
               const uint64_t *tc, const Fr &z, uint64_t n, hipStream_t s);
void k_perm_numden(uint64_t *num, uint64_t *den, const PermArgs &a, uint64_t n, hipStream_t s);
void k_lookup_nd(uint64_t *num, uint64_t *den, const uint64_t *f, const uint64_t *t,
                 const uint64_t *h1, const uint64_t *h2, const Fr &delta, const Fr &eps, uint64_t n,
                 hipStream_t s);
void k_mul_inplace(uint64_t *a, const uint64_t *b, uint64_t n, hipStream_t s);
bool k_any_nonzero(const uint64_t *v, uint64_t words, DevBuf &scratch, hipStream_t s);
void k_any_nonzero_n(const uint64_t *v, uint64_t words, uint64_t stride, int cnt, bool *nz, DevBuf &scratch,
                     hipStream_t s);
bool k_any_diff(const uint64_t *a, const uint64_t *b, uint64_t words, DevBuf &scratch, hipStream_t s);
void k_hash_words(const uint64_t *a, uint64_t words, DevBuf &scratch, hipStream_t s, uint64_t out[2]);
bool k_pack_affine(const uint8_t *src, uint64_t n, uint64_t stride, uint64_t x_off, uint64_t y_off,
                   uint64_t inf_off, uint64_t *dst, DevBuf &scratch, hipStream_t s);
void k_affine(uint64_t *out, const uint64_t *in, const Fr &a, const Fr &b, uint64_t n, hipStream_t s);
void k_quotient(const QuotArgs &q, uint64_t N8, uint64_t *out, hipStream_t s);
void k_lincomb(const LinArgs &a, uint64_t n, uint64_t *out, hipStream_t s);
void k_widgets(const WidgetArgs &g, uint64_t N8, uint64_t *out, hipStream_t s);
bool combine_split(pnp_ctx *ctx, const uint64_t *t, const uint64_t *f, uint64_t n, uint64_t *h1,
                   uint64_t *h2, hipStream_t s);
void k_proof_marker(hipStream_t s);

}
```

zprize23-gpu-submission_amd/csrc/protocol.hip:

```cpp
#include "pnp_internal.h"
#include "protocol.h"
#include "widgets.cuh"
#include "fr29.cuh"
#include <vector>

namespace pnp {

static inline uint32_t nblk(uint64_t threads, uint32_t bs = 256) {
    return (uint32_t)((threads + bs - 1) / bs);
}

__global__ void k_compress4_(uint64_t *out, const uint64_t *t0, const uint64_t *t1,
                             const uint64_t *t2, const uint64_t *t3, Fr z, uint64_t n) {
    uint64_t i = blockIdx.x * (uint64_t)blockDim.x + threadIdx.x;
    if (i >= n) return;
    Fr acc = load_fr(t3, i);
    acc = acc * z + load_fr(t2, i);
    acc = acc * z + load_fr(t1, i);
    acc = acc * z + load_fr(t0, i);
    store_fr(out, i, acc);
}
void k_compress4(uint64_t *out, const uint64_t *t0, const uint64_t *t1, const uint64_t *t2,
                 const uint64_t *t3, const Fr &z, uint64_t n, hipStream_t s) {
    hipLaunchKernelGGL(k_compress4_, dim3(nblk(n)), dim3(256), 0, s, out, t0, t1, t2, t3, z, n);
// ... 68 lines not shown
    store_fr(den, i, d);
}
void k_lookup_nd(uint64_t *num, uint64_t *den, const uint64_t *f, const uint64_t *t,
                 const uint64_t *h1, const uint64_t *h2, const Fr &delta, const Fr &eps, uint64_t n,
                 hipStream_t s) {
    hipLaunchKernelGGL(k_lookup_nd_, dim3(nblk(n)), dim3(256), 0, s, num, den, f, t, h1, h2, delta, eps,
                       n);
    PNP_HIP(hipGetLastError());
}

__global__ void k_mul_inplace_(uint64_t *a, const uint64_t *b, uint64_t n) {
    uint64_t i = blockIdx.x * (uint64_t)blockDim.x + threadIdx.x;
    if (i < n) store_fr(a, i, load_fr(a, i) * load_fr(b, i));
}
void k_mul_inplace(uint64_t *a, const uint64_t *b, uint64_t n, hipStream_t s) {
    hipLaunchKernelGGL(k_mul_inplace_, dim3(nblk(n)), dim3(256), 0, s, a, b, n);
    PNP_HIP(hipGetLastError());
}

__global__ __launch_bounds__(256) void k_any_nonzero_(const uint64_t *v, uint64_t words, uint64_t stride,
                                                      unsigned *flag) {
    const ulonglong2 *p = reinterpret_cast<const ulonglong2 *>(v + stride * blockIdx.y);
    const uint64_t pairs = words / 2;
    uint64_t acc = 0;
    for (uint64_t i = blockIdx.x * (uint64_t)blockDim.x + threadIdx.x; i < pairs;
         i += (uint64_t)gridDim.x * blockDim.x) {
        const ulonglong2 x = p[i];
        acc |= x.x | x.y;
    }
    if (blockIdx.x == 0 && threadIdx.x == 0 && (words & 1)) acc |= v[stride * blockIdx.y + words - 1];
    if (__any(acc != 0) && (threadIdx.x & 63) == 0) atomicOr(flag + blockIdx.y, 1u);
}
void k_any_nonzero_n(const uint64_t *v, uint64_t words, uint64_t stride, int cnt, bool *nz, DevBuf &scratch,
                     hipStream_t s) {
    if (scratch.bytes < 4 * (size_t)cnt + 16) scratch.alloc(4 * (size_t)cnt + 16);
    unsigned *flag = static_cast<unsigned *>(scratch.p);
    PNP_HIP(hipMemsetAsync(flag, 0, 4 * (size_t)cnt, s));
    if (words) {
        uint64_t blocks = (words / 2 + 255) / 256;
        if (blocks > 2048) blocks = 2048;
        if (blocks == 0) blocks = 1;
        hipLaunchKernelGGL(k_any_nonzero_, dim3((uint32_t)blocks, (uint32_t)cnt), dim3(256), 0, s, v, words,
                           stride, flag);
        PNP_HIP(hipGetLastError());
    }
    std::vector<unsigned> h(cnt);
    PNP_HIP(hipMemcpyAsync(h.data(), flag, 4 * (size_t)cnt, hipMemcpyDeviceToHost, s));
    PNP_HIP(hipStreamSynchronize(s));
    for (int k = 0; k < cnt; k++) nz[k] = h[k] != 0;
}
bool k_any_nonzero(const uint64_t *v, uint64_t words, DevBuf &scratch, hipStream_t s) {
    bool nz = false;
    if (words) k_any_nonzero_n(v, words, words, 1, &nz, scratch, s);
    return nz;
}

__global__ void k_any_diff_(const uint64_t *a, const uint64_t *b, uint64_t words, unsigned *flag) {
    uint64_t i = blockIdx.x * (uint64_t)blockDim.x + threadIdx.x;
    uint64_t stride = (uint64_t)gridDim.x * blockDim.x;
    uint64_t acc = 0;
    for (; i < words; i += stride) acc |= a[i] ^ b[i];
    if (__any(acc != 0) && (threadIdx.x & 63) == 0) atomicOr(flag, 1u);
}
bool k_any_diff(const uint64_t *a, const uint64_t *b, uint64_t words, DevBuf &scratch, hipStream_t s) {
    if (!words) return false;
    if (scratch.bytes < 16) scratch.alloc(16);
    unsigned *flag = static_cast<unsigned *>(scratch.p);
    PNP_HIP(hipMemsetAsync(flag, 0, 4, s));
    uint64_t blocks = (words + 255) / 256;
    if (blocks > 4096) blocks = 4096;
    hipLaunchKernelGGL(k_any_diff_, dim3((uint32_t)blocks), dim3(256), 0, s, a, b, words, flag);
    PNP_HIP(hipGetLastError());
    unsigned h = 0;
    PNP_HIP(hipMemcpyAsync(&h, flag, 4, hipMemcpyDeviceToHost, s));
    PNP_HIP(hipStreamSynchronize(s));
    return h != 0;
}

__device__ __forceinline__ uint64_t dmum(uint64_t a, uint64_t b) {
    return a * b ^ __umul64hi(a, b);
}
__global__ void k_hash_words_(const uint64_t *a, uint64_t words, unsigned long long *out) {
    uint64_t i = blockIdx.x * (uint64_t)blockDim.x + threadIdx.x;
    const uint64_t stride = (uint64_t)gridDim.x * blockDim.x;
    uint64_t h0 = 0, h1 = 0;
    for (; i < words; i += stride) {
// ... 234 lines not shown
    w.d_next = load_fr(g.w8[3], nx);
    w.q_l = load_fr(g.q_l, i);
    w.q_r = load_fr(g.q_r, i);
    w.q_c = load_fr(g.q_c, i);
    Fr acc = Fr::zero();
    if (g.sel[0]) acc += load_fr(g.sel[0], i) * w_range(g.sep[0], w);
    if (g.sel[1]) acc += load_fr(g.sel[1], i) * w_logic(g.sep[1], w);
    if (g.sel[2]) acc += load_fr(g.sel[2], i) * w_fbsm(g.sep[2], w);
    if (g.sel[3]) acc += load_fr(g.sel[3], i) * w_cadd(g.sep[3], w);
    store_fr(out, i, load_fr(out, i) + acc * load_fr(g.vh_inv, i));
}
void k_widgets(const WidgetArgs &g, uint64_t N8, uint64_t *out, hipStream_t s) {
    hipLaunchKernelGGL(k_widgets_, dim3(nblk(N8)), dim3(256), 0, s, g, N8, out);
    PNP_HIP(hipGetLastError());
}

__global__ __launch_bounds__(256) void k_lincomb_(LinArgs a, uint64_t n, uint64_t *out) {
    uint64_t i = blockIdx.x * (uint64_t)blockDim.x + threadIdx.x;
    if (i >= n) return;
    Fr acc = Fr::zero();
    int k = 0;
    for (; k + 1 < a.k; k += 2) acc += fr_mul2(load_fr(a.p[k], i), a.s[k], load_fr(a.p[k + 1], i), a.s[k + 1]);
    if (k < a.k) acc += load_fr(a.p[k], i) * a.s[k];
    store_fr(out, i, acc);
}
void k_lincomb(const LinArgs &a, uint64_t n, uint64_t *out, hipStream_t s) {
    hipLaunchKernelGGL(k_lincomb_, dim3(nblk(n)), dim3(256), 0, s, a, n, out);
    PNP_HIP(hipGetLastError());
}

}

namespace pnp {
__global__ void k_proof_begin() {}
void k_proof_marker(hipStream_t s) {
    hipLaunchKernelGGL(k_proof_begin, dim3(1), dim3(1), 0, s);
    PNP_HIP(hipGetLastError());
}
}
```

zprize23-gpu-submission_amd/csrc/prover.cpp:

```cpp
#include <chrono>
#include <string.h>
#include "context.h"
#include "protocol.h"
#include "transcript.h"
#include "widgets.cuh"
#include <algorithm>

namespace pnp {

Fr fr_from_u64(uint64_t x) {
    Fr r = Fr::zero();
    r.v[0] = (uint32_t)x;
    r.v[1] = (uint32_t)(x >> 32);
    return to_mont(r);
}

Fr root_of_unity(uint32_t lg) {
    const uint64_t root32[4] = {13381757501831005802ULL, 6564924994866501612ULL,
                                789602057691799140ULL, 6625830629041353339ULL};
    return pow_u64(from_u64_limbs<FrP>(root32), 1ULL << (32 - lg));
}

namespace {

// ... 102 lines not shown
            }
            v.emplace_back(opt->pi_pos[k], to_mont(from_u64_limbs<FrP>(opt->pi_canon + 4 * k)));
        }
        std::sort(v.begin(), v.end(), [](const auto &a, const auto &b) { return a.first < b.first; });
        for (size_t k = 0; k < v.size(); k++) {
            if (k && v[k].first == v[k - 1].first) {
                set_error("public input position %llu given twice", (unsigned long long)v[k].first);
                return PNP_E_ARG;
            }
            if (v[k].second.is_zero()) continue;
            pi_pos.push_back(v[k].first);
            pi_val.push_back(v[k].second);
        }
    }
    if (ctx->defer_tables < 0) ctx->defer_tables = ctx->msm.world <= 1 ? 1 : 0;
    const bool bg_mode = ctx->msm.world <= 1 && tables_bg_enabled();
    ctx->defer_now = ctx->defer_tables == 1 && (bg_mode || ctx->proofs_started == 0);
    ctx->proofs_started++;
    ctx->tables_wanted = false;
    struct DeferScope {
        pnp_ctx *c;
        ~DeferScope() { c->defer_now = false; }
    } defer_scope{ctx};
    if (!ctx->hbm_checked) {
        hbm_budget(ctx);
        ctx->hbm_checked = true;
    }
    ctx->msm.batch_seq = 0;
    const uint64_t N8 = 8 * n, ng = asg ? ctx->wm_gates : cs->n;
    const ProverKeyC &pk = ctx->pk_dev;
    Timer tm(ctx);
    auto &nt = ctx->ntt;
    auto alg = [&](double elems) { ctx->ktimer.credit("proof_alg_bytes", 32.0 * elems); };
    k_proof_marker(s);
    ntt_warm(nt, lg, s);
    const int world = ctx->msm.world;
    if (ctx->pk_blk_world != world || ctx->pk_blk_rank != ctx->msm.rank) {
        set_error("sharding changed after pnp_load_prover_key");
        return PNP_E_ARG;
    }
    const int mb0 = ctx->pk_mb0, nb = ctx->pk_nb;
    const bool dist = nb < 8;
    const uint64_t NB = (uint64_t)nb * n;
    uint64_t q0 = 0, q1 = n;
    if (dist) msm_point_range(n, ctx->msm.rank, world, q0, q1);
    const uint64_t len = q1 - q0;
    static const bool overlap = getenv("PNP_NO_OVERLAP") == nullptr;
    hipStream_t s_lo = overlap ? ctx->side_stream() : s;
    static const int quot_blocks = [] {
        const char *e = getenv("PNP_QUOT_BLOCKS");
        int v = e ? atoi(e) : 6;
        return v < 6 ? 6 : v > 8 ? 8 : v;
    }();
    int nbq = dist ? nb : quot_blocks;
    const bool q29 = ctx->pk_q29;
    auto lde_on = [&](hipStream_t st, const uint64_t *coeffs, uint64_t *dst, bool f29) {
        lde_blocks(nt, coeffs, dst, lg, mb0, nbq, st, f29);
    };
    auto fork = [&]() {
        if (!overlap) return;
        PNP_HIP(hipEventRecord(ctx->ev_fork, s));
        PNP_HIP(hipStreamWaitEvent(s_lo, ctx->ev_fork, 0));
    };

    uint64_t *wsc[4], *wpoly[4];
    for (int j = 0; j < 4; j++) {
        wsc[j] = ctx->buf("wsc" + std::to_string(j), n);
// ... 49 lines not shown
    uint64_t *w8buf[4];
    for (int j = 0; j < 4; j++) w8buf[j] = ctx->buf("w8_" + std::to_string(j), NB);
    CommitmentC *wc[4] = {&out->a_comm, &out->b_comm, &out->c_comm, &out->d_comm};
    if (lag) {
        fork();
        for (int j = 0; j < 4; j++) ntt_run(nt, wpoly[j], lg, true, false, s_lo, wsc[j]);
        for (int j = 0; j < 4; j++) lde_on(s_lo, wpoly[j], w8buf[j], q29);
        if (overlap) PNP_HIP(hipEventRecord(ctx->ev_w8, s_lo));
        alg(4.0 * 2 * n + 4.0 * (1 + nbq) * n);
        tm.mark("r1_intt");
        const uint64_t *sc[4] = {wsc[0], wsc[1], wsc[2], wsc[3]};
        if (commit_wires_grouped(ctx, sc, n, wc)) alg(4.0 * n * 72 / 32);
        else commit_evals_batch(ctx, sc, 4, n, wc);
    } else {
        for (int j = 0; j < 4; j++) ntt_run(nt, wpoly[j], lg, true, false, s, wsc[j]);
        alg(4.0 * 2 * n + 4.0 * (1 + nbq) * n);
        tm.mark("r1_intt");
        fork();
        for (int j = 0; j < 4; j++) lde_on(s_lo, wpoly[j], w8buf[j], q29);
        if (overlap) PNP_HIP(hipEventRecord(ctx->ev_w8, s_lo));
        const uint64_t *sc[4] = {wpoly[0], wpoly[1], wpoly[2], wpoly[3]};
        commit_affine_batch(ctx, sc, 4, n, wc);
    }
    append_comm(tr, "w_l", *wc[0]);
    append_comm(tr, "w_r", *wc[1]);
    append_comm(tr, "w_o", *wc[2]);
    append_comm(tr, "w_4", *wc[3]);
    tm.mark("r1_commit");

    Fr zeta = tr.challenge_scalar("zeta");
    tr.append_scalar("zeta", zeta);
    uint64_t *tc = ctx->buf("tc", n), *table_poly = ctx->buf("table_poly", n);
    k_compress4(tc, pk.table1, pk.table2, pk.table3, pk.table4, zeta, n, s);
    const bool table_zero = !k_any_nonzero(tc, 4 * n, ctx->scratch_b, s);
    uint64_t *fc = ctx->buf("fc", n), *f_poly = ctx->buf("f_poly", n);
    const uint64_t *wconst[4] = {wsc[0], wsc[1], wsc[2], wsc[3]};
    k_query_f(fc, qlk, qlk_rows, wconst, tc, zeta, n, s);
    const bool f_zero = !k_any_nonzero(fc, 4 * n, ctx->scratch_b, s);
    alg(5.0 * n + n + ng + n + n);
    if (!table_zero) ntt_run(nt, table_poly, lg, true, false, s, tc);
    if (!f_zero) ntt_run(nt, f_poly, lg, true, false, s, fc);
    const bool h_zero = f_zero && table_zero;
    uint64_t *h1 = ctx->buf("h1", n), *h2 = ctx->buf("h2", n);
    uint64_t *h1_poly = ctx->buf("h1_poly", n), *h2_poly = ctx->buf("h2_poly", n);
    {
        const uint64_t *sc[3];
        CommitmentC *oc[3];
        int nc = 0;
        if (f_zero) {
            set_infinity(&out->f_comm);
        } else {
            sc[nc] = f_poly;
            oc[nc++] = &out->f_comm;
        }
        if (h_zero) {
            PNP_HIP(hipMemsetAsync(h1, 0, 32 * n, s));
            PNP_HIP(hipMemsetAsync(h2, 0, 32 * n, s));
            alg(2.0 * n);
            set_infinity(&out->h_1_comm);
            set_infinity(&out->h_2_comm);
        } else {
            if (!combine_split(ctx, tc, fc, n, h1, h2, s)) {
                set_error("lookup: a query value is not in the lookup table (Error::ElementNotIndexed)");
                return PNP_E_ARG;
            }
            ntt_run(nt, h1_poly, lg, true, false, s, h1);
            ntt_run(nt, h2_poly, lg, true, false, s, h2);
            sc[nc] = h1_poly;
            oc[nc++] = &out->h_1_comm;
            sc[nc] = h2_poly;
            oc[nc++] = &out->h_2_comm;
        }
        if (nc) commit_affine_batch(ctx, sc, nc, n, oc);
    }
    append_comm(tr, "f", out->f_comm);
    append_comm(tr, "h1", out->h_1_comm);
    append_comm(tr, "h2", out->h_2_comm);
    tm.mark("r2_lookup");

    Fr beta = tr.challenge_scalar("beta");
    tr.append_scalar("beta", beta);
    Fr gamma = tr.challenge_scalar("gamma");
    tr.append_scalar("gamma", gamma);
    Fr delta = tr.challenge_scalar("delta");
    tr.append_scalar("delta", delta);
    Fr eps = tr.challenge_scalar("epsilon");
    tr.append_scalar("epsilon", eps);
    if (beta == gamma || beta == delta || beta == eps || gamma == delta || gamma == eps ||
        delta == eps) {
        set_error("challenges must be different");
        return PNP_E_ARG;
// ... 13 lines not shown
    pa.omega = root_of_unity(lg);
    pa.tw = ntt_twiddles(nt, lg, false, s);
    uint64_t *num = ctx->buf("num", n), *den = ctx->buf("den", n);
    uint64_t *z_poly = ctx->buf("z_poly", n);
    k_perm_numden(num, den, pa, n, s);
    k_batch_inverse(den, n, ctx->scratch_a, s);
    k_mul_inplace(num, den, n, s);
    k_prefix_product(num, n, ctx->scratch_a, s);
    alg(10.0 * n + 2.0 * n + 3.0 * n + 2.0 * n);
    alg(2.0 * n + (1.0 + nbq) * n);
    uint64_t *z8 = ctx->buf("z8", NB);
    if (lag) {
        fork();
        ntt_run(nt, z_poly, lg, true, false, s_lo, num);
        lde_on(s_lo, z_poly, z8, q29);
        if (overlap) PNP_HIP(hipEventRecord(ctx->ev_z8, s_lo));
        tm.mark("r3_z");
        const uint64_t *sc[1] = {num};
        CommitmentC *oc[1] = {&out->z_comm};
        if (commit_z_grouped(ctx, num, n, &out->z_comm)) alg(1.0 * n * 72 / 32);
        else commit_evals_batch(ctx, sc, 1, n, oc);
    } else {
        ntt_run(nt, z_poly, lg, true, false, s, num);
        tm.mark("r3_z");
        fork();
        lde_on(s_lo, z_poly, z8, q29);
        if (overlap) PNP_HIP(hipEventRecord(ctx->ev_z8, s_lo));
        commit_affine(ctx, z_poly, n, &out->z_comm);
    }
    append_comm(tr, "z", out->z_comm);
    uint64_t *z2_poly = ctx->buf("z2_poly", n);
    const bool z2_one = h_zero;
    if (z2_one) {
        uint64_t one[4];
        to_u64_limbs(Fr::one(), one);
        PNP_HIP(hipMemsetAsync(z2_poly, 0, 32 * n, s));
        PNP_HIP(hipMemcpyAsync(z2_poly, one, 32, hipMemcpyHostToDevice, s));
        PNP_HIP(hipStreamSynchronize(s));
    } else {
        if (lag && overlap) PNP_HIP(hipStreamWaitEvent(s, ctx->ev_z8, 0));
        k_lookup_nd(num, den, fc, tc, h1, h2, delta, eps, n, s);
        k_batch_inverse(den, n, ctx->scratch_a, s);
        k_mul_inplace(num, den, n, s);
        k_prefix_product(num, n, ctx->scratch_a, s);
        ntt_run(nt, z2_poly, lg, true, false, s, num);
    }
    const Fr n_inv = inverse(fr_from_u64(n));
    const bool closed = ctx->pk_std_coset;
    const bool pi_closed = closed && pi_pos.size() == 1;
    uint64_t *pi_poly = nullptr;
    if (pi_pos.size() == 1 && !closed) {
        pi_poly = ctx->buf("pi_poly", n);
        Fr w_inv_pos = pow_u64(inverse(root_of_unity(lg)), pi_pos[0]);
        k_geometric(pi_poly, n, pi_val[0] * n_inv, w_inv_pos, s);
    } else if (pi_pos.size() > 1) {
        pi_poly = ctx->buf("pi_poly", n);
        PNP_HIP(hipMemsetAsync(pi_poly, 0, 32 * n, s));
        std::vector<uint64_t> limbs(4 * pi_val.size());
        for (size_t k = 0; k < pi_val.size(); k++) to_u64_limbs(pi_val[k], &limbs[4 * k]);
        for (size_t k = 0; k < pi_val.size(); k++)
            PNP_HIP(hipMemcpyAsync(pi_poly + 4 * pi_pos[k], &limbs[4 * k], 32, hipMemcpyHostToDevice, s));
        PNP_HIP(hipStreamSynchronize(s));
        ntt_run(nt, pi_poly, lg, true, false, s);
    }
    if (pi_closed && ctx->pk_pinv_pos != pi_pos[0]) {
        ctx->pk_pinv_pos = ~0ULL;
        if (ctx->pk_pinv.bytes < 32 * NB) ctx->pk_pinv.alloc(32 * NB);
        Fr wpos = pow_u64(root_of_unity(lg), pi_pos[0]);
        k_affine(ctx->pk_pinv.u64(), ctx->blk("lin"), Fr::one(), neg(wpos), NB, s);
        k_batch_inverse(ctx->pk_pinv.u64(), NB, ctx->scratch_a, s);
        ctx->pk_pinv_pos = pi_pos[0];
    }
    tm.mark("r3_z2_pi");

    const Transcript tr3 = tr;
    for (;;) {
        const uint64_t NBq = (uint64_t)nbq * n;
        Fr alpha = tr.challenge_scalar("alpha");
        tr.append_scalar("alpha", alpha);
        Fr range_c = tr.challenge_scalar("range separation challenge");
        tr.append_scalar("range seperation challenge", range_c);
        Fr logic_c = tr.challenge_scalar("logic separation challenge");
        tr.append_scalar("logic seperation challenge", logic_c);
        Fr fixed_c = tr.challenge_scalar("fixed base separation challenge");
        tr.append_scalar("fixed base separation challenge", fixed_c);
        Fr var_c = tr.challenge_scalar("variable base separation challenge");
        tr.append_scalar("variable base separation challenge", var_c);
        Fr lsep = tr.challenge_scalar("lookup separation challenge");
        tr.append_scalar("lookup separation challenge", lsep);

        QuotArgs q;
        auto lde = [&](const uint64_t *coeffs, uint64_t *dst) { lde_on(s, coeffs, dst, false); };
        for (int j = 0; j < 4; j++) q.w8[j] = w8buf[j];
        uint64_t *z28 = ctx->buf("z28", NB);
        q.z8 = z8;
        q.pi8 = nullptr;
        q.l18 = q.l1v = q.pinv = nullptr;
        if (closed) q.l1v = ctx->blk("l1v");
        if (pi_closed) {
            q.pinv = ctx->pk_pinv.u64();
            q.c_pi = pi_val[0] * pow_u64(root_of_unity(lg), pi_pos[0]) * n_inv;
        } else if (pi_poly) {
            uint64_t *pi8 = ctx->buf("pi8", NB);
            lde_on(s, pi_poly, pi8, q29);
            q.pi8 = pi8;
        }
        q.z28 = nullptr;
        if (!z2_one) {
            lde(z2_poly, z28);
// ... 116 lines not shown
            WidgetArgs g;
            for (int j = 0; j < 4; j++) g.w8[j] = q.w8[j];
            g.q_l = q.q_l;
            g.q_r = q.q_r;
            g.q_c = q.q_c;
            g.vh_inv = q.vh_inv;
            g.sel[0] = ctx->blk("range");
            g.sel[1] = ctx->blk("logic");
            g.sel[2] = ctx->blk("fixed_add");
            g.sel[3] = ctx->blk("var_add");
            g.sep[0] = range_c;
            g.sep[1] = logic_c;
            g.sep[2] = fixed_c;
            g.sep[3] = var_c;
            g.n = n;
            g.lg_n = lg;
            k_widgets(g, NBq, t_blk, s);
        }
        {
            const uint64_t *arrs[] = {q.w8[0], q.w8[1], q.w8[2], q.w8[3], q.q_m, q.q_l, q.q_r, q.q_o,
                                      q.q_4, q.q_c, q.q_hl, q.q_hr, q.q_h4, q.q_arith, q.pi8, q.lin,
                                      q.z8, q.sig[0], q.sig[1], q.sig[2], q.sig[3], q.f8,
                                      q.t8, q.h18, q.h28, q.q_lookup, q.z28, q.l18, q.vh_inv, q.l1v, q.pinv};
            int nread = 0;
            for (const uint64_t *a : arrs) nread += a != nullptr;
            ctx->ktimer.end("quotient", s, qe0, 32.0 * (double)NBq * (nread + 1));
            alg((double)NBq * (nread + 1));
        }
        tm.mark("r4_quotient");
        intt_blocks(nt, t_blk, lg, mb0, nbq, s);
        alg(2.0 * NBq + 2.0 * NBq);
        uint64_t *t_poly = ctx->buf("t_poly", 8 * len);
        const int npieces = dist ? 8 : nbq;
        unsigned *t_nz = reinterpret_cast<unsigned *>(ctx->buf("t_nz", 1));
        PNP_HIP(hipMemsetAsync(t_nz, 0, 4, s));
        if (!dist) {
            t_combine_blocks(nt, t_blk, nbq, t_poly, lg, t_nz, s);
        } else {
            const uint64_t slot = (uint64_t)nb * len * 32;
            if (!ctx->msm.alltoall || ctx->msm.a2a_bytes < 2 * slot * world) {
                set_error("round-4 all-to-all buffer missing or < %llu B",
                          (unsigned long long)(2 * slot * world));
                return PNP_E_ARG;
            }
            uint64_t *a2a = ctx->msm.a2a;
            for (int r = 0; r < world; r++) {
                uint64_t r0, r1;
                msm_point_range(n, r, world, r0, r1);
                for (int b = 0; b < nb; b++)
                    PNP_HIP(hipMemcpyAsync(a2a + 4 * ((uint64_t)(r * nb + b) * len), t_blk + 4 * ((uint64_t)b * n + r0),
                                           32 * len, hipMemcpyDeviceToDevice, s));
            }
            ex_fence(ctx->msm, s);
            int rc = ctx->msm.alltoall(ctx->msm.a2a_user, slot);
            if (rc != 0) {
                set_error("round-4 all-to-all callback failed (%d)", rc);
                return PNP_E_DEVICE;
            }
            t_combine(nt, a2a + 4 * (uint64_t)nb * len * world, len, q0, t_poly, lg, t_nz, s);
        }
        tm.mark("r4_intt8");
        CommitmentC *tcm[8] = {&out->t_1_comm, &out->t_2_comm, &out->t_3_comm, &out->t_4_comm,
                               &out->t_5_comm, &out->t_6_comm, &out->t_7_comm, &out->t_8_comm};
        {
            const uint64_t *sc[9];
            CommitmentC *oc[9];
            int nc = 0;
            uint64_t nz[8];
            {
                unsigned bits = 0;
                PNP_HIP(hipMemcpyAsync(&bits, t_nz, 4, hipMemcpyDeviceToHost, s));
                PNP_HIP(hipStreamSynchronize(s));
                for (int k = 0; k < 8; k++) nz[k] = k < npieces && ((bits >> k) & 1);
            }
            if (dist) {
                std::vector<uint64_t> all = shard_allgather(ctx, nz, 8, PNP_EX_TAG_T_FLAGS);
                for (int k = 0; k < 8; k++) {
                    nz[k] = 0;
                    for (int r = 0; r < world; r++) nz[k] |= all[8 * r + k];
                }
            }
            for (int k = 0; k < 8; k++) {
                if (!nz[k]) {
                    set_infinity(tcm[k]);
                    continue;
                }
                sc[nc] = t_poly + 4 * (uint64_t)k * len;
                oc[nc++] = tcm[k];
            }
            if (z2_one) {
                uint64_t g0[12];
                PNP_HIP(hipMemcpyAsync(g0, ctx->ck_dev, sizeof g0, hipMemcpyDeviceToHost, s));
                PNP_HIP(hipStreamSynchronize(s));
                memcpy(out->z_2_comm.x, g0, 48);
                memcpy(out->z_2_comm.y, g0 + 6, 48);
            } else if (dist) {
                commit_affine(ctx, z2_poly, n, &out->z_2_comm);
            } else {
                sc[nc] = z2_poly;
                oc[nc++] = &out->z_2_comm;
            }
            commit_affine_batch(ctx, sc, nc, n, oc, dist);
        }
        const char *tl[8] = {"t_1", "t_2", "t_3", "t_4", "t_5", "t_6", "t_7", "t_8"};
        for (int k = 0; k < 8; k++) append_comm(tr, tl[k], *tcm[k]);
        tm.mark("r4_commit");
        ctx->ktimer.collect();

        Fr zc = tr.challenge_scalar("z");
        tr.append_scalar("z", zc);
        Fr omega = root_of_unity(lg);
        Fr zw = zc * omega;
        Fr vh = pow_u64(zc, n) - Fr::one();
        Fr zn = vh + Fr::one();
        Fr l1e = vh * inverse(fr_from_u64(n) * (zc - Fr::one()));
        ProofEvaluationsC *ev = &out->evaluations;
        {
            const uint64_t eo = 4 * q0;
            const uint64_t *pz[12] = {wpoly[0] + eo, wpoly[1] + eo, wpoly[2] + eo, wpoly[3] + eo,
                                      pk.left_sigma_coeffs + eo, pk.right_sigma_coeffs + eo,
                                      pk.out_sigma_coeffs + eo, pk.q_arith_coeffs + eo, pk.q_c_coeffs + eo,
                                      pk.q_l_coeffs + eo, pk.q_r_coeffs + eo, pk.q_hl_coeffs + eo};
            Fr rz[12];
            const uint64_t *pz2[2] = {pk.q_hr_coeffs + eo, pk.q_h4_coeffs + eo};
            Fr rz2[2];
            const uint64_t *pw[4] = {z_poly + eo, wpoly[0] + eo, wpoly[1] + eo, wpoly[3] + eo};
            Fr rw[4];
            const EvalSet sets[3] = {{pz, 12, zc, rz}, {pz2, 2, zc, rz2}, {pw, 4, zw, rw}};
// ... 255 lines not shown
```

zprize23-gpu-submission_amd/csrc/wires.hip:

```cpp
#include <hipcub/hipcub.hpp>
#include <algorithm>
#include "context.h"
#include "ec.cuh"
#include "protocol.h"

namespace pnp {

namespace {

inline uint32_t nblk(uint64_t threads, uint32_t bs = 256) { return (uint32_t)((threads + bs - 1) / bs); }

__device__ __forceinline__ bool fr_eq(const uint64_t *a, const uint64_t *b) {
    return a[0] == b[0] && a[1] == b[1] && a[2] == b[2] && a[3] == b[3];
}

__global__ void k_wb_keys(const uint64_t *idv, uint64_t N, uint64_t *key, uint32_t *pos) {
    const uint64_t p = blockIdx.x * (uint64_t)blockDim.x + threadIdx.x;
    if (p >= N) return;
    key[p] = idv[4 * p];
    pos[p] = (uint32_t)p;
}

struct SigmaPtrs {
    const uint64_t *s[4];
// ... 414 lines not shown
        }
        const bool all = all_ranks_ok(ctx, fits);
        if (!all) {
            ctx->wb = pnp_ctx::WireBases{};
            wb.built = true;
            wb.n = n;
            wb.pk_gen = ctx->pk_gen;
            ctx->hbm_groups_off = true;
        } else if (ctx->msm.world > 1) {
            const bool w = all_ranks_ok(ctx, wb.wires_ok), z = all_ranks_ok(ctx, wb.z_ok);
            if (w != wb.wires_ok || z != wb.z_ok) {
                set_error("wire groups: the ranks built different groups from one prover key");
                throw Error(PNP_E_DEVICE);
            }
        }
    }
    return wb.ok;
}

}

void wire_bases_reset(pnp_ctx *ctx) { ctx->wb = pnp_ctx::WireBases{}; }
void wire_bases_build(pnp_ctx *ctx, uint64_t n) {
    if (groups_enabled() && !ctx->hbm_groups_off) wire_bases_ready(ctx, n);
}
bool wire_groups_enabled() { return groups_enabled(); }

bool commit_wires_grouped(pnp_ctx *ctx, const uint64_t *const *d_evals, uint64_t n, CommitmentC *const *out) {
    if (!groups_enabled() || ctx->hbm_groups_off || !lagrange_table(ctx, n) || !wire_bases_ready(ctx, n) ||
        !ctx->wb.wires_ok)
        return false;
    auto &wb = ctx->wb;
    hipStream_t s = ctx->stream;
    uint32_t *flag = static_cast<uint32_t *>(wb.flag.p);
    PNP_HIP(hipMemsetAsync(flag, 0, 4, s));
    WirePtrs wp{};
    for (int j = 0; j < 4; j++) {
        wp.w[j] = d_evals[j];
        if (wb.ident[j]) continue;
        wp.grp[j] = static_cast<const uint32_t *>(wb.grp[j].p);
        wp.rep[j] = static_cast<const uint32_t *>(wb.rep[j].p);
        wp.scal[j] = wb.scal[j].u64();
    }
    hipLaunchKernelGGL(k_wb_gather, dim3(nblk(n), 4), dim3(256), 0, s, wp, n, flag);
    PNP_HIP(hipGetLastError());
    uint32_t hflag = 0;
    PNP_HIP(hipMemcpyAsync(&hflag, flag, 4, hipMemcpyDeviceToHost, s));
    PNP_HIP(hipStreamSynchronize(s));
    if (hflag) {
        if (ctx->ktimer.enabled) ctx->ktimer.credit("wire_group_fallback", 1);
        return false;
    }
    const uint64_t *sc[4];
    MsmSegs segs;
    segs.n_table = wb.total;
    segs.sliced = wb.sliced;
    segs.c = wb.c;
    for (int j = 0; j < 4; j++) {
        sc[j] = wb.ident[j] ? d_evals[j] : wb.scal[j].u64();
        segs.off[j] = wb.off[j];
    }
    std::vector<uint64_t> xyzz(4 * 24);
    msm_run_batch(ctx->msm, nullptr, sc, 4, wb.len, xyzz.data(), s, wb.table.u64(), false, &segs);
    std::vector<uint64_t> aff(4 * 12);
    xyzz_to_affine_batch_host(xyzz.data(), 4, aff.data());
    for (int b = 0; b < 4; b++) {
        memcpy(out[b]->x, &aff[12 * b], 48);
        memcpy(out[b]->y, &aff[12 * b + 6], 48);
    }
    if (ctx->ktimer.enabled) ctx->ktimer.credit("wire_groups_used", 1);
    return true;
}

bool commit_z_grouped(pnp_ctx *ctx, const uint64_t *d_z, uint64_t n, CommitmentC *out) {
    if (!z_groups_enabled() || ctx->hbm_groups_off || !lagrange_table(ctx, n) || !wire_bases_ready(ctx, n) ||
        !ctx->wb.z_ok)
        return false;
    auto &wb = ctx->wb;
    hipStream_t s = ctx->stream;
    uint32_t *flag = static_cast<uint32_t *>(wb.flag.p);
    PNP_HIP(hipMemsetAsync(flag, 0, 4, s));
    WirePtrs wp{};
    wp.w[0] = d_z;
    wp.grp[0] = static_cast<const uint32_t *>(wb.grp[4].p);
    wp.rep[0] = static_cast<const uint32_t *>(wb.rep[4].p);
    wp.scal[0] = wb.scal[4].u64();
    hipLaunchKernelGGL(k_wb_gather, dim3(nblk(n), 1), dim3(256), 0, s, wp, n, flag);
    PNP_HIP(hipGetLastError());
    uint32_t hflag = 0;
    PNP_HIP(hipMemcpyAsync(&hflag, flag, 4, hipMemcpyDeviceToHost, s));
    PNP_HIP(hipStreamSynchronize(s));
    if (hflag) {
        if (ctx->ktimer.enabled) ctx->ktimer.credit("z_group_fallback", 1);
        return false;
    }
    const uint64_t *sc[1] = {wb.scal[4].u64()};
    MsmSegs segs;
    segs.n_table = wb.total;
    segs.sliced = wb.sliced;
    segs.c = wb.c;
    segs.off[0] = wb.off[4];
    uint64_t xyzz[24], aff[12];
    msm_run_batch(ctx->msm, nullptr, sc, 1, wb.len, xyzz, s, wb.table.u64(), false, &segs);
    xyzz_to_affine_batch_host(xyzz, 1, aff);
    memcpy(out->x, aff, 48);
    memcpy(out->y, aff + 6, 48);
    if (ctx->ktimer.enabled) ctx->ktimer.credit("z_groups_used", 1);
    return true;
}

}
```

zprize23-gpu-submission_amd/pnp/__init__.py:

```python
import ctypes as C
import os

from . import abi

_HERE = os.path.dirname(os.path.abspath(__file__))
LIB_PATH = os.environ.get("PNP_PLONK_LIB",
                          os.path.join(os.path.dirname(_HERE), "lib", "libpnp_plonk.so"))
_LIB = None

PNP_OK = 0
ERRORS = {-1: "PNP_E_ARG", -2: "PNP_E_DEVICE", -3: "PNP_E_NOKEY", -4: "PNP_E_ENVELOPE",
          -5: "PNP_E_NOMEM"}

SYMBOLS = ("gen_proof", "pnp_last_error", "pnp_ctx_create", "pnp_ctx_destroy",
           "pnp_load_prover_key", "pnp_load_prover_key_coeffs", "pnp_load_commit_key", "pnp_prove", "pnp_prove_ex",
           "pnp_last_stage_times",
           "pnp_kernel_timing", "pnp_kernel_stats", "pnp_kernel_bytes", "pnp_set_msm_shard",
           "pnp_set_exchange_a2a",
           "pnp_sync", "pnp_ntt", "pnp_coset_lde8", "pnp_commit", "pnp_commit_ck", "pnp_commit_evals", "pnp_poly_eval",
           "pnp_poly_div_linear", "pnp_prefix_product", "pnp_batch_inverse",
           "pnp_synth_random_fr", "pnp_synth_srs", "pnp_synth_coset_consts", "pnp_synth_circuit",
           "pnp_synth_merkle", "pnp_load_commit_key_strided", "pnp_proof_infinity_mask",
           "pnp_set_exchange_v", "pnp_commit_segments", "pnp_hbm_usage",
           "pnp_ctx_stream", "pnp_set_exchange_ordered", "pnp_v1_context",
           "pnp_preprocess", "pnp_wire_sigma",
           "pnp_load_wire_map", "pnp_gather_witness", "pnp_prove_assignment")


ALLGATHER_FN = C.CFUNCTYPE(C.c_int, C.c_void_p, C.c_uint64)
ALLTOALL_FN = C.CFUNCTYPE(C.c_int, C.c_void_p, C.c_uint64)
ALLTOALLV_FN = C.CFUNCTYPE(C.c_int, C.c_void_p, C.POINTER(C.c_uint64), C.POINTER(C.c_uint64))


class PnpError(RuntimeError):
    pass


def load(path: str = LIB_PATH):
    global _LIB
    if _LIB is not None:
        return _LIB
    if not os.path.exists(path):
        raise PnpError(f"{path} not built (run __graft_entry__.build() or make -C csrc)")
    try:
        import torch
    except ImportError:
        pass
    lib = C.CDLL(path)
    vp, u64, i32 = C.c_void_p, C.c_uint64, C.c_int
    lib.gen_proof.argtypes = [abi.CircuitC, abi.ProverKeyC, abi.CommitKeyC]
    lib.gen_proof.restype = abi.ProofC
    lib.pnp_v1_context.restype = vp
    lib.pnp_last_error.restype = C.c_char_p
    lib.pnp_ctx_create.argtypes = [i32, C.POINTER(vp)]
    lib.pnp_ctx_destroy.argtypes = [vp]
    lib.pnp_ctx_destroy.restype = None
    lib.pnp_load_prover_key.argtypes = [vp, C.POINTER(abi.ProverKeyC), u64, i32]
    lib.pnp_load_prover_key_coeffs.argtypes = [vp, C.POINTER(abi.ProverKeyC), u64, i32]
    lib.pnp_load_commit_key.argtypes = [vp, C.POINTER(abi.CommitKeyC), u64, i32]
    lib.pnp_preprocess.argtypes = [vp, C.POINTER(abi.CircuitDesc), i32, C.POINTER(abi.VerifierKey)]
    lib.pnp_wire_sigma.argtypes = [vp, C.c_void_p * 4, u64, u64, C.c_uint32, vp, C.POINTER(C.c_void_p * 4)]
    lib.pnp_prove.argtypes = [vp, C.POINTER(abi.CircuitC), i32, C.POINTER(abi.ProofC)]
    lib.pnp_prove_ex.argtypes = [vp, C.POINTER(abi.CircuitC), i32, u64, vp, vp, C.c_char_p,
                                 C.POINTER(abi.ProofC)]
    for name, argtypes in abi.ASSIGNMENT_ARGTYPES.items():
        getattr(lib, name).argtypes = argtypes
    lib.pnp_last_stage_times.argtypes = [vp, C.POINTER(C.c_double), C.POINTER(C.c_char_p), i32]
    lib.pnp_kernel_timing.argtypes = [vp, i32]
    lib.pnp_kernel_stats.argtypes = [vp, C.c_char_p, C.POINTER(C.c_double), C.POINTER(C.c_int)]
    lib.pnp_kernel_bytes.argtypes = [vp, C.c_char_p, C.POINTER(C.c_double)]
    lib.pnp_set_msm_shard.argtypes = [vp, i32, i32, ALLGATHER_FN, vp, vp, u64]
    lib.pnp_set_exchange_a2a.argtypes = [vp, ALLTOALL_FN, vp, vp, u64]
    lib.pnp_set_exchange_v.argtypes = [vp, ALLTOALLV_FN, vp, vp, vp, u64]
    lib.pnp_sync.argtypes = [vp]
    lib.pnp_ntt.argtypes = [vp, vp, C.c_uint32, i32, i32]
    lib.pnp_coset_lde8.argtypes = [vp, vp, vp, C.c_uint32]
    lib.pnp_commit.argtypes = [vp, vp, vp, u64, C.POINTER(abi.CommitmentC)]
    lib.pnp_commit_ck.argtypes = [vp, vp, u64, C.POINTER(abi.CommitmentC)]
    lib.pnp_commit_evals.argtypes = [vp, vp, u64, C.POINTER(abi.CommitmentC)]
    lib.pnp_hbm_usage.argtypes = [vp, C.POINTER(u64)]
    lib.pnp_ctx_stream.argtypes = [vp, C.POINTER(vp)]
    lib.pnp_set_exchange_ordered.argtypes = [vp, i32]
    lib.pnp_commit_segments.argtypes = [vp, vp, u64, i32, C.POINTER(u64), C.POINTER(vp), u64,
                                        C.POINTER(abi.CommitmentC)]
    lib.pnp_poly_eval.argtypes = [vp, vp, u64, vp, vp]
    lib.pnp_poly_div_linear.argtypes = [vp, vp, u64, vp]
    lib.pnp_prefix_product.argtypes = [vp, vp, u64]
    lib.pnp_batch_inverse.argtypes = [vp, vp, u64]
    lib.pnp_synth_random_fr.argtypes = [vp, vp, u64, u64]
    lib.pnp_synth_srs.argtypes = [vp, vp, u64, vp]
    lib.pnp_synth_coset_consts.argtypes = [vp, vp, vp, C.c_uint32]
    lib.pnp_synth_circuit.argtypes = [vp, C.c_void_p * 4, C.c_void_p * 9, C.c_void_p * 4, u64, u64,
                                      u64, vp]
    lib.pnp_synth_merkle.argtypes = [vp, C.c_uint32, vp, vp, vp, vp, C.c_void_p * 4, C.c_void_p * 9,
                                     C.c_void_p * 4, u64, vp]
    lib.pnp_load_commit_key_strided.argtypes = [vp, vp, u64, C.POINTER(abi.AffineLayout), i32]
    lib.pnp_proof_infinity_mask.argtypes = [C.POINTER(abi.ProofC)]
    for name in SYMBOLS:
        if name.startswith("pnp_") and name not in ("pnp_last_error", "pnp_ctx_destroy", "pnp_v1_context"):
            getattr(lib, name).restype = C.c_int if name != "pnp_last_error" else C.c_char_p
    lib.pnp_proof_infinity_mask.restype = C.c_uint32
    _LIB = lib
    return lib


def infinity_mask(proof: abi.ProofC) -> int:
    return int(load().pnp_proof_infinity_mask(C.byref(proof)))


def infinity_flags(proof: abi.ProofC) -> dict:
    m = infinity_mask(proof)
    return {name: bool((m >> k) & 1) for k, name in enumerate(abi.PROOF_COMMITMENTS)}


def check(rc: int, what: str = ""):
    if rc != PNP_OK:
        msg = load().pnp_last_error()
        raise PnpError(f"{what}: {ERRORS.get(rc, rc)}: {msg.decode() if msg else ''}")


class Context:

    def __init__(self, device: int = 0):
        self.lib = load()
        h = C.c_void_p()
        check(self.lib.pnp_ctx_create(device, C.byref(h)), "pnp_ctx_create")
        self.h = h

    def close(self):
        if self.h:
            self.lib.pnp_ctx_destroy(self.h)
# ... 131 lines not shown
        check(self.lib.pnp_sync(self.h), "pnp_sync")

    def ntt(self, addr: int, lg_n: int, inverse: bool = False, coset: bool = False):
        check(self.lib.pnp_ntt(self.h, C.c_void_p(addr), lg_n, int(inverse), int(coset)), "pnp_ntt")

    def coset_lde8(self, src: int, dst: int, lg_n: int):
        check(self.lib.pnp_coset_lde8(self.h, C.c_void_p(src), C.c_void_p(dst), lg_n), "pnp_coset_lde8")

    def commit(self, points: int, scalars: int, n: int) -> abi.CommitmentC:
        out = abi.CommitmentC()
        check(self.lib.pnp_commit(self.h, C.c_void_p(points), C.c_void_p(scalars), n, C.byref(out)),
              "pnp_commit")
        return out

    def commit_ck(self, scalars: int, n: int) -> abi.CommitmentC:
        out = abi.CommitmentC()
        check(self.lib.pnp_commit_ck(self.h, C.c_void_p(scalars), n, C.byref(out)), "pnp_commit_ck")
        return out

    def commit_evals(self, evals: int, n: int) -> abi.CommitmentC:
        out = abi.CommitmentC()
        check(self.lib.pnp_commit_evals(self.h, C.c_void_p(evals), n, C.byref(out)), "pnp_commit_evals")
        return out

    def commit_segments(self, points: int, n_points: int, seg_off, scalars, n: int):
        B = len(seg_off)
        offs = (C.c_uint64 * B)(*seg_off)
        sc = (C.c_void_p * B)(*scalars)
        out = (abi.CommitmentC * B)()
        check(self.lib.pnp_commit_segments(self.h, C.c_void_p(points), n_points, B, offs, sc, n, out),
              "pnp_commit_segments")
        return list(out)

    def gather_witness(self, var, n_gates: int, values: int, n_vars: int, lg_n: int, w):
        V = (C.c_void_p * 4)(*[a or None for a in var])
        W = (C.c_void_p * 4)(*[a or None for a in w])
        check(self.lib.pnp_gather_witness(self.h, V, n_gates, C.c_void_p(values or None), n_vars, lg_n, W),
              "pnp_gather_witness")

    def poly_eval(self, addr: int, n: int, x_limbs):
        x = (C.c_uint64 * 4)(*x_limbs)
        out = (C.c_uint64 * 4)()
        check(self.lib.pnp_poly_eval(self.h, C.c_void_p(addr), n, x, out), "pnp_poly_eval")
        return list(out)

    def poly_div_linear(self, addr: int, n: int, z_limbs):
        z = (C.c_uint64 * 4)(*z_limbs)
        check(self.lib.pnp_poly_div_linear(self.h, C.c_void_p(addr), n, z), "pnp_poly_div_linear")

    def prefix_product(self, addr: int, n: int):
        check(self.lib.pnp_prefix_product(self.h, C.c_void_p(addr), n), "pnp_prefix_product")

    def batch_inverse(self, addr: int, n: int):
        check(self.lib.pnp_batch_inverse(self.h, C.c_void_p(addr), n), "pnp_batch_inverse")

    def random_fr(self, addr: int, n: int, seed: int):
        check(self.lib.pnp_synth_random_fr(self.h, C.c_void_p(addr), n, seed), "pnp_synth_random_fr")

    def srs(self, addr: int, n: int, tau_limbs):
        t = (C.c_uint64 * 4)(*tau_limbs)
        check(self.lib.pnp_synth_srs(self.h, C.c_void_p(addr), n, t), "pnp_synth_srs")

    def synth_circuit(self, w, sel, sigma, n: int, n_gates: int, pi_pos: int, pi_limbs):
        W = (C.c_void_p * 4)(*w)
        S = (C.c_void_p * 9)(*sel)
        G = (C.c_void_p * 4)(*sigma)
# ... 15 lines not shown
```

Baseline: 0.1239.

## Fold small memsets and host syncs into a shared control block

```diff
diff --git a/include/pnp_plonk.h b/include/pnp_plonk.h
--- a/include/pnp_plonk.h
+++ b/include/pnp_plonk.h
@@ -250,6 +250,8 @@
                         const uint64_t *seg_off, const uint64_t *const *d_scalars, uint64_t n,
                         CommitmentC *out);
 
+int pnp_msm_work_counters(pnp_ctx *ctx, uint64_t ref[2], uint64_t dev[2]);
+
 int pnp_wire_sigma(pnp_ctx *ctx, const uint32_t *const d_var[4], uint64_t n_gates, uint64_t n_vars,
                    uint32_t lg_n, uint32_t *d_next, uint64_t *const d_sigma[4]);
 
diff --git a/zprize23-gpu-submission_amd/csrc/abi.cpp b/zprize23-gpu-submission_amd/csrc/abi.cpp
--- a/zprize23-gpu-submission_amd/csrc/abi.cpp
+++ b/zprize23-gpu-submission_amd/csrc/abi.cpp
@@ -823,6 +823,15 @@
             memcpy(out[b].x, &aff[12 * b], 48);
             memcpy(out[b].y, &aff[12 * b + 6], 48);
         }
+    });
+}
+
+int pnp_msm_work_counters(pnp_ctx *ctx, uint64_t ref[2], uint64_t dev[2]) {
+    if (!ctx || !ref || !dev) return PNP_E_ARG;
+    PNP_TRY({
+        unsigned long long r[2], d[2];
+        msm_work_recount(ctx->msm, ctx->stream, r, d);
+        for (int k = 0; k < 2; k++) ref[k] = r[k], dev[k] = d[k];
     });
 }
 
@@ -1504,6 +1513,11 @@
 
 namespace {
 
+void fetch_ck_g0(pnp_ctx *ctx) {
+    PNP_HIP(hipMemcpyAsync(ctx->ck_g0, ctx->ck_dev, sizeof ctx->ck_g0, hipMemcpyDeviceToHost, ctx->stream));
+    PNP_HIP(hipStreamSynchronize(ctx->stream));
+}
+
 void adopt_ck(pnp_ctx *ctx, pnp::DevBuf &up, uint64_t n_points) {
     const bool same = ctx->ck_owned.p && ctx->ck_dev == ctx->ck_owned.u64() && ctx->ck_points == n_points &&
                       !pnp::k_any_diff(up.u64(), ctx->ck_owned.u64(), 12 * n_points, ctx->scratch_b, ctx->stream);
@@ -1512,6 +1526,7 @@
         std::swap(ctx->ck_owned, up);
         ctx->ck_dev = ctx->ck_owned.u64();
         pnp::ck_derived_reset(ctx);
+        fetch_ck_g0(ctx);
     }
     ctx->ck_points = n_points;
     ctx->ck_loaded = true;
@@ -1536,7 +1551,10 @@
             ctx->ck_owned.release();
             ctx->ck_dev = ck->powers_of_g;
             ctx->ck_points = n_points;
-            if (!same) pnp::ck_derived_reset(ctx);
+            if (!same) {
+                pnp::ck_derived_reset(ctx);
+                fetch_ck_g0(ctx);
+            }
             ctx->ck_hash[0] = h[0];
             ctx->ck_hash[1] = h[1];
             ctx->ck_hash_valid = true;
diff --git a/zprize23-gpu-submission_amd/csrc/context.h b/zprize23-gpu-submission_amd/csrc/context.h
--- a/zprize23-gpu-submission_amd/csrc/context.h
+++ b/zprize23-gpu-submission_amd/csrc/context.h
@@ -56,6 +56,10 @@
     uint64_t ck_points = 0;
     pnp::DevBuf ck_owned;
     const uint64_t *ck_dev = nullptr;
+    uint64_t ck_g0[12] = {};
+    unsigned *proof_ctl = nullptr;
+    const uint64_t *z2_one_at = nullptr;
+    uint64_t z2_one_n = 0;
     uint64_t ck_hash[2] = {0, 0};
     bool ck_hash_valid = false;
     pnp::DevBuf ck_table;
diff --git a/zprize23-gpu-submission_amd/csrc/msm.hip b/zprize23-gpu-submission_amd/csrc/msm.hip
--- a/zprize23-gpu-submission_amd/csrc/msm.hip
+++ b/zprize23-gpu-submission_amd/csrc/msm.hip
@@ -84,9 +84,16 @@
     return (((uint64_t)(b / nbl) * nv + v) * nbl + b % nbl) * nch + ch;
 }
 
+__device__ __forceinline__ void hist_total_slot(uint32_t *counts, int NBc, int nch, uint32_t *ctl, int ctl_words) {
+    if (blockIdx.x != 0 || blockIdx.y != 0) return;
+    if (threadIdx.x == 0) counts[(uint64_t)gridDim.y * NBc * nch] = 0;
+    if (ctl && (int)threadIdx.x < ctl_words) ctl[threadIdx.x] = 0;
+}
+
 __global__ __launch_bounds__(1024) void k_coarse_hist(const uint32_t *keys, KeyRows kr, int fb,
                                                       int NBc, uint64_t chunk, int nch,
-                                                      uint32_t *counts, int wmaj = 1) {
+                                                      uint32_t *counts, int wmaj = 1, uint32_t *ctl = nullptr,
+                                                      int ctl_words = 0) {
     __shared__ uint32_t hist[1 << SORT_CB];
     const int v = blockIdx.y, ch = blockIdx.x;
     for (int b = threadIdx.x; b < NBc; b += blockDim.x) hist[b] = 0;
@@ -114,6 +121,7 @@
     }
     __syncthreads();
     for (int b = threadIdx.x; b < NBc; b += blockDim.x) counts[cidx(v, gridDim.y, b, NBc, wmaj, ch, nch)] = hist[b];
+    hist_total_slot(counts, NBc, nch, ctl, ctl_words);
 }
 
 struct ScalarPtrs {
@@ -123,7 +131,7 @@
 __global__ __launch_bounds__(1024) void k_digits_hist(ScalarPtrs sp, uint64_t n, int c, int W, int top_sh, int fb,
                                                       int NBc,
                                                       uint64_t chunk, int nch, uint32_t *keys, uint32_t *counts,
-                                                      int wmaj = 1) {
+                                                      int wmaj = 1, uint32_t *ctl = nullptr, int ctl_words = 0) {
     __shared__ uint32_t hist[1 << SORT_CB];
     const int v = blockIdx.y, ch = blockIdx.x;
     for (int b = threadIdx.x; b < NBc; b += blockDim.x) hist[b] = 0;
@@ -136,6 +144,7 @@
         });
     __syncthreads();
     for (int b = threadIdx.x; b < NBc; b += blockDim.x) counts[cidx(v, gridDim.y, b, NBc, wmaj, ch, nch)] = hist[b];
+    hist_total_slot(counts, NBc, nch, ctl, ctl_words);
 }
 
 __global__ __launch_bounds__(256) void k_scan_tiles(uint32_t *d, uint64_t n, uint32_t *tile_sums) {
@@ -494,6 +503,7 @@
     for (int f = threadIdx.x; f < NF; f += blockDim.x) h[f] = ps + lofs[f];
     __syncthreads();
     for (int f = threadIdx.x; f < NF; f += blockDim.x) bstart[p * NF + f] = h[f];
+    if (p + 1 == gridDim.x && threadIdx.x == 0) bstart[(p + 1) * NF] = pe;
     constexpr int PER = TILE_F / 1024;
     uint32_t ne[PER], nf[PER];
     auto load_tile = [&](uint32_t tb) {
@@ -846,7 +856,7 @@
                                                       const uint32_t *offs, uint64_t U, uint64_t nthr, uint32_t S,
                                                       uint32_t *buckets, uint32_t *head,
                                                       uint32_t *tail, uint32_t *tailb, uint32_t *redo,
-                                                      uint32_t *nredo, uint32_t *tlist) {
+                                                      MsmCtl *ctl, uint32_t *tlist, uint32_t count_work) {
 #if PNP_ACC_GLDS == 1
     __shared__ uint4 stage[4 * 7 * 64];
     __shared__ uint32_t sidx[4 * 64];
@@ -870,6 +880,7 @@
     bool first = offs[cur] < lo;
     uint32_t next = offs[cur + 1];
     bool ok = true, fresh = true;
+    uint32_t npieces = 1;
     Xyzz29 acc;
 #if PNP_ACC_GLDS == 1
     uint32_t e = sorted[lo];
@@ -886,6 +897,7 @@
             ok &= store29(first ? head + 56 * t : buckets + 56 * cur, acc);
             first = false;
             fresh = true;
+            npieces++;
             cur = next_bucket(offs, 1, U, cur + 1, k, next);
         }
 #if PNP_ACC_GLDS == 2
@@ -937,14 +949,23 @@
         const int leader = __ffsll((unsigned long long)m) - 1;
         const uint32_t below = __builtin_amdgcn_mbcnt_hi((uint32_t)(m >> 32), __builtin_amdgcn_mbcnt_lo((uint32_t)m, 0u));
         uint32_t base = 0;
-        if (below == 0) base = atomicAdd(tlist, (uint32_t)__popcll(m));
+        if (below == 0) base = atomicAdd(&ctl->ntail, (uint32_t)__popcll(m));
         base = __shfl(base, leader);
-        tlist[1 + base + below] = (uint32_t)t;
-    }
-    if (!ok) redo[atomicAdd(nredo, 1u)] = (uint32_t)t;
-}
-
-constexpr int WCTR_SLOTS = 64;
+        tlist[base + below] = (uint32_t)t;
+    }
+    if (!ok) redo[atomicAdd(&ctl->nredo, 1u)] = (uint32_t)t;
+    if (count_work) {
+        uint32_t wsum = 0;
+        for (int bit = 0; __ballot(npieces != 0); bit++, npieces >>= 1)
+            wsum += (uint32_t)__popcll(__ballot(npieces & 1u)) << bit;
+        const uint64_t live = __ballot(true);
+        const uint32_t lane = __builtin_amdgcn_mbcnt_hi(~0u, __builtin_amdgcn_mbcnt_lo(~0u, 0u));
+        if (lane == (uint32_t)(__ffsll((unsigned long long)live) - 1))
+            atomicAdd(&ctl->wctr[1 + ((t >> 6) & (WCTR_SLOTS - 1))], (unsigned long long)wsum);
+        if (t == 0) ctl->wctr[0] = total;
+    }
+}
+
 __global__ __launch_bounds__(1024) void k_count_pieces(const uint32_t *offs, uint64_t WB, uint64_t nthr, uint32_t S,
                                                        unsigned long long *ctr) {
     S = acc_seg(offs, WB, nthr, S);
@@ -1118,6 +1139,9 @@
     int nv;
 };
 
+static size_t ctl_bytes(const MsmWork &wk) { return wk.timer ? sizeof(MsmCtl) : offsetof(MsmCtl, wctr); }
+constexpr size_t CTL_BUF_BYTES = sizeof(MsmCtl) + (size_t)MSM_BATCH_MAX * 48 * 8;
+
 static void sort_group(MsmWork &wk, MsmGroup &gb, const uint32_t *keys, const GroupPlan &gp,
                        const MsmCfg &g, hipStream_t s, const uint64_t *const *scalars = nullptr) {
     const int nv = gp.nv;
@@ -1141,17 +1165,21 @@
     uint32_t *counts = static_cast<uint32_t *>(gb.counts.p);
     uint32_t *bstart = static_cast<uint32_t *>(gb.offsets.p);
     dim3 grid((uint32_t)nch, (uint32_t)nv);
+    need(gb.ctl, CTL_BUF_BYTES);
+    uint32_t *ctl = static_cast<uint32_t *>(gb.ctl.p);
+    const int ctl_words = (int)(ctl_bytes(wk) / 4);
     if (scalars) {
         ScalarPtrs sp{};
         for (int v = 0; v < nv; v++) sp.p[v] = scalars[v];
         hipLaunchKernelGGL(k_digits_hist, grid, dim3(1024), 0, s, sp, n, g.c, g.W, g.top_sh, fb, NBc, chunk, nch,
-                           const_cast<uint32_t *>(keys), counts, 1);
+                           const_cast<uint32_t *>(keys), counts, 1, ctl, ctl_words);
     } else {
-        hipLaunchKernelGGL(k_coarse_hist, grid, dim3(1024), 0, s, keys, gp.kr, fb, NBc, chunk, nch, counts);
+        hipLaunchKernelGGL(k_coarse_hist, grid, dim3(1024), 0, s, keys, gp.kr, fb, NBc, chunk, nch, counts, 1, ctl,
+                           ctl_words);
     }
     PNP_HIP(hipGetLastError());
+    gb.ctl_cleared = true;
     const uint64_t ncount = nbins * nch;
-    PNP_HIP(hipMemsetAsync(counts + ncount, 0, 4, s));
     scan_u32(counts, ncount + 1, gb.scan_tmp, s);
     uint32_t *ent = static_cast<uint32_t *>(gb.ent.p);
     uint16_t *fk = static_cast<uint16_t *>(gb.fkey.p);
@@ -1161,7 +1189,6 @@
     hipLaunchKernelGGL(k_fine_sort, dim3((uint32_t)nbins), dim3(1024), 0, s, ent, fk, counts, nch, fb,
                        bstart, static_cast<uint32_t *>(gb.sorted.p));
     PNP_HIP(hipGetLastError());
-    PNP_HIP(hipMemcpyAsync(bstart + WB, counts + ncount, 4, hipMemcpyDeviceToDevice, s));
 }
 
 static uint32_t acc_segment(uint64_t nent, bool folded) {
@@ -1200,29 +1227,32 @@
     const uint32_t S = acc_segment(nent, table != nullptr);
     const uint64_t nthr = (nent + S - 1) / S;
     if (table) {
-        need(gb.seg, (WB + 2 * nthr) * 224 + nthr * 4 + (nthr + 1) * 4);
+        need(gb.seg, (WB + 2 * nthr) * 224 + nthr * 4 + nthr * 4);
         uint32_t *bk29 = static_cast<uint32_t *>(gb.seg.p);
         uint32_t *head = bk29 + 56 * WB, *tail = head + 56 * nthr, *tailb = tail + 56 * nthr;
         uint32_t *tlist = tailb + nthr;
-        PNP_HIP(hipMemsetAsync(tlist, 0, 4, s));
-        need(gb.redo, nthr * 4 + 16);
-        uint32_t *nredo = static_cast<uint32_t *>(gb.redo.p), *redo = nredo + 4;
-        PNP_HIP(hipMemsetAsync(nredo, 0, 4, s));
+        need(gb.redo, nthr * 4);
+        uint32_t *redo = static_cast<uint32_t *>(gb.redo.p);
+        need(gb.ctl, CTL_BUF_BYTES);
+        MsmCtl *ctl = gb.ctl_dev();
+        const bool count_work = wk.timer != nullptr;
+        if (!gb.ctl_cleared) PNP_HIP(hipMemsetAsync(ctl, 0, ctl_bytes(wk), s));
+        gb.ctl_cleared = false;
         const uint32_t *t29 = reinterpret_cast<const uint32_t *>(table);
         const uint32_t blocks = (uint32_t)((nthr + 255) / 256);
         hipLaunchKernelGGL(k_accumulate29, dim3(blocks), dim3(256), 0, s, t29, sorted, bstart, WB, nthr, S, bk29,
-                           head, tail, tailb, redo, nredo, tlist);
+                           head, tail, tailb, redo, ctl, tlist, count_work ? 1u : 0u);
         PNP_HIP(hipGetLastError());
+        gb.wctr_live = count_work;
         hipLaunchKernelGGL(k_accumulate_redo, dim3((uint32_t)std::min<uint64_t>((nthr + 63) / 64, 1024)), dim3(64), 0, s, t29,
-                           sorted, bstart, WB, nthr, S, bk29, head, tail, redo, nredo);
+                           sorted, bstart, WB, nthr, S, bk29, head, tail, redo, &ctl->nredo);
         PNP_HIP(hipGetLastError());
-        need(gb.exc, 16);
-        PNP_HIP(hipMemsetAsync(gb.exc.p, 0, 4, s));
         gb.S = S;
         gb.pieces = (uint32_t)(nent / WB / S + 1);
         gb.nthr = nthr;
-        need(gb.heavy, (WB + 1) * 4);
-        msm_merge_pieces29(bstart, WB, S, nthr, tailb, tlist, bk29, head, tail, static_cast<uint32_t *>(gb.exc.p),
+        gb.WB = WB;
+        need(gb.heavy, WB * 4);
+        msm_merge_pieces29(bstart, WB, S, nthr, tailb, &ctl->ntail, tlist, bk29, head, tail, &ctl->exc, &ctl->nheavy,
                            static_cast<uint32_t *>(gb.heavy.p), s);
     } else {
         need(gb.seg, nthr * 2 * 24 * 8);
@@ -1235,38 +1265,56 @@
     if (wk.timer) {
         wk.timer->end("msm_accumulate", s, ev0, alg_bytes);
         wk.timer->credit("msm_entries_dense", (double)nent);
-        if (table) {
-            need(gb.wctr, 8 * (1 + WCTR_SLOTS));
-            PNP_HIP(hipMemsetAsync(gb.wctr.p, 0, 8 * (1 + WCTR_SLOTS), s));
-            hipLaunchKernelGGL(k_count_pieces, dim3((uint32_t)((WB + 1023) / 1024)), dim3(1024), 0, s, bstart, WB, nthr, S,
-                               static_cast<unsigned long long *>(gb.wctr.p));
-            PNP_HIP(hipGetLastError());
-            gb.wctr_live = true;
-        }
-    }
-}
-
-static void wctr_fetch(MsmGroup &gb, hipStream_t s) {
-    if (gb.wctr_live) PNP_HIP(hipMemcpyAsync(gb.wctr_h, gb.wctr.p, 8 * (1 + WCTR_SLOTS), hipMemcpyDeviceToHost, s));
+    }
+}
+
+static void ctl_fetch(MsmGroup &gb, hipStream_t s) {
+    PNP_HIP(hipMemcpyAsync(&gb.ctl_h, gb.ctl.p, gb.wctr_live ? sizeof(MsmCtl) : offsetof(MsmCtl, wctr),
+                           hipMemcpyDeviceToHost, s));
 }
 static void wctr_credit(MsmWork &wk, MsmGroup &gb) {
     if (!gb.wctr_live) return;
     gb.wctr_live = false;
     if (!wk.timer) return;
     unsigned long long pieces = 0;
-    for (int k = 1; k <= WCTR_SLOTS; k++) pieces += gb.wctr_h[k];
-    wk.timer->credit("msm_entries", (double)gb.wctr_h[0]);
-    wk.timer->credit("msm_madds", (double)(gb.wctr_h[0] - pieces));
-}
-
+    for (int k = 1; k <= WCTR_SLOTS; k++) pieces += gb.ctl_h.wctr[k];
+    wk.timer->credit("msm_entries", (double)gb.ctl_h.wctr[0]);
+    wk.timer->credit("msm_madds", (double)(gb.ctl_h.wctr[0] - pieces));
+}
+
+void msm_work_recount(MsmWork &wk, hipStream_t s, unsigned long long ref[2], unsigned long long dev[2]) {
+    MsmGroup &gb = wk.grp[0];
+    if (!gb.ctl.p || !gb.WB) {
+        set_error("msm_work_recount: no folded accumulation has run");
+        throw Error(PNP_E_ARG);
+    }
+    DevBuf tmp(8 * (1 + WCTR_SLOTS));
+    unsigned long long h[2][1 + WCTR_SLOTS];
+    PNP_HIP(hipMemsetAsync(tmp.p, 0, tmp.bytes, s));
+    hipLaunchKernelGGL(k_count_pieces, dim3((uint32_t)((gb.WB + 1023) / 1024)), dim3(1024), 0, s,
+                       static_cast<const uint32_t *>(gb.offsets.p), gb.WB, gb.nthr, gb.S,
+                       static_cast<unsigned long long *>(tmp.p));
+    PNP_HIP(hipGetLastError());
+    PNP_HIP(hipMemcpyAsync(h[0], tmp.p, sizeof h[0], hipMemcpyDeviceToHost, s));
+    PNP_HIP(hipMemcpyAsync(h[1], gb.ctl_dev()->wctr, sizeof h[1], hipMemcpyDeviceToHost, s));
+    PNP_HIP(hipStreamSynchronize(s));
+    for (int j = 0; j < 2; j++) {
+        unsigned long long *o = j ? dev : ref;
+        o[0] = h[j][0], o[1] = 0;
+        for (int k = 1; k <= WCTR_SLOTS; k++) o[1] += h[j][k];
+    }
+}
+
+static bool ctl_results_ok(const GroupPlan &gp) { return gp.nv <= MSM_BATCH_MAX; }
 static const uint64_t *reduce_group(MsmGroup &gb, const GroupPlan &gp, const MsmCfg &g, hipStream_t s,
-                                    bool folded) {
+                                    bool folded, bool to_ctl = false) {
     const uint64_t WB = (uint64_t)gp.nv * g.NB;
     uint64_t *bk = gb.buckets.u64();
     if (folded)
         return msm_reduce29(static_cast<const uint32_t *>(gb.seg.p), static_cast<const uint32_t *>(gb.offsets.p),
                             (uint64_t)gp.nv, g.NB,
-                            reinterpret_cast<uint32_t *>(bk), static_cast<uint32_t *>(gb.exc.p), s);
+                            reinterpret_cast<uint32_t *>(bk), &gb.ctl_dev()->exc, s,
+                            to_ctl ? reinterpret_cast<uint64_t *>(gb.ctl_dev() + 1) : nullptr);
     return msm_reduce(bk, (uint64_t)gp.nv, g.NB, bk + WB * 24, s);
 }
 
@@ -1362,7 +1410,7 @@
     if (ng == 1) {
         sort_group(wk, wk.grp[0], keys, gp[0], g, s, fuse ? d_scalars : nullptr);
         accumulate_group(wk, wk.grp[0], gp[0], g, pts, table, s);
-        res[0] = reduce_group(wk.grp[0], gp[0], g, s, folded);
+        res[0] = reduce_group(wk.grp[0], gp[0], g, s, folded, folded && ctl_results_ok(gp[0]));
     } else {
         if (!wk.s2) PNP_HIP(hipStreamCreateWithFlags(&wk.s2, hipStreamNonBlocking));
         hipEvent_t evD = ev_get(wk, 0), evS1 = ev_get(wk, 1), evA0 = ev_get(wk, 2), evR0 = ev_get(wk, 3);
@@ -1374,26 +1422,35 @@
         accumulate_group(wk, wk.grp[0], gp[0], g, pts, table, s);
         PNP_HIP(hipEventRecord(evA0, s));
         PNP_HIP(hipStreamWaitEvent(wk.s2, evA0, 0));
-        res[0] = reduce_group(wk.grp[0], gp[0], g, wk.s2, folded);
+        res[0] = reduce_group(wk.grp[0], gp[0], g, wk.s2, folded, folded && ctl_results_ok(gp[0]));
         PNP_HIP(hipEventRecord(evR0, wk.s2));
         PNP_HIP(hipStreamWaitEvent(s, evS1, 0));
         accumulate_group(wk, wk.grp[1], gp[1], g, pts, table, s);
-        res[1] = reduce_group(wk.grp[1], gp[1], g, s, folded);
+        res[1] = reduce_group(wk.grp[1], gp[1], g, s, folded, folded && ctl_results_ok(gp[1]));
         PNP_HIP(hipStreamWaitEvent(s, evR0, 0));
     }
-    std::vector<uint64_t> win[2];
+    std::vector<uint64_t> win[2], both[2];
     uint32_t exc[2] = {0, 0}, nredo[2] = {0, 0};
     for (int k = 0; k < ng; k++) {
         win[k].resize((size_t)gp[k].nv * 24);
+        if (folded && ctl_results_ok(gp[k])) {
+            both[k].resize(sizeof(MsmCtl) / 8 + win[k].size());
+            PNP_HIP(hipMemcpyAsync(both[k].data(), wk.grp[k].ctl.p, both[k].size() * 8, hipMemcpyDeviceToHost, s));
+            continue;
+        }
         PNP_HIP(hipMemcpyAsync(win[k].data(), res[k], win[k].size() * 8, hipMemcpyDeviceToHost, s));
-        if (folded) {
-            PNP_HIP(hipMemcpyAsync(&exc[k], wk.grp[k].exc.p, 4, hipMemcpyDeviceToHost, s));
-            PNP_HIP(hipMemcpyAsync(&nredo[k], wk.grp[k].redo.p, 4, hipMemcpyDeviceToHost, s));
-            wctr_fetch(wk.grp[k], s);
-        }
+        if (folded) ctl_fetch(wk.grp[k], s);
     }
     PNP_HIP(hipStreamSynchronize(s));
-    for (int k = 0; k < ng; k++) wctr_credit(wk, wk.grp[k]);
+    for (int k = 0; k < ng && folded; k++) {
+        if (!both[k].empty()) {
+            wk.grp[k].ctl_h = *reinterpret_cast<const MsmCtl *>(both[k].data());
+            std::copy(both[k].begin() + sizeof(MsmCtl) / 8, both[k].end(), win[k].begin());
+        }
+        exc[k] = wk.grp[k].ctl_h.exc;
+        nredo[k] = wk.grp[k].ctl_h.nredo;
+        wctr_credit(wk, wk.grp[k]);
+    }
     if (wk.timer) wk.timer->credit("msm_redo_lanes", (double)nredo[0] + nredo[1]);
     for (int k = 0; k < ng; k++) {
         if (!exc[k]) continue;
@@ -1569,18 +1626,18 @@
         GroupPlan gp;
         gp.kr = kr;
         gp.nv = B;
+        gb.ctl_cleared = false;
         accumulate_group(wk, gb, gp, gl, nullptr, table, s, W * cap, (double)W * cap * 128.0 / g.W);
         const uint64_t *res = reduce_group(gb, gp, gl, s, true);
         std::vector<uint64_t> ts((size_t)B * 48);
         uint32_t exc = 0, nredo = 0, fl[2] = {0, 0};
         std::vector<uint32_t> dc(W);
         PNP_HIP(hipMemcpyAsync(ts.data(), res, ts.size() * 8, hipMemcpyDeviceToHost, s));
-        PNP_HIP(hipMemcpyAsync(&exc, gb.exc.p, 4, hipMemcpyDeviceToHost, s));
-        PNP_HIP(hipMemcpyAsync(&nredo, gb.redo.p, 4, hipMemcpyDeviceToHost, s));
         PNP_HIP(hipMemcpyAsync(fl, flags, 8, hipMemcpyDeviceToHost, s));
         PNP_HIP(hipMemcpyAsync(dc.data(), dcnt, 4 * W, hipMemcpyDeviceToHost, s));
-        wctr_fetch(gb, s);
+        ctl_fetch(gb, s);
         PNP_HIP(hipStreamSynchronize(s));
+        exc = gb.ctl_h.exc, nredo = gb.ctl_h.nredo;
         wk.slot_runs++;
         if (fl[0]) {
             gb.wctr_live = false;
@@ -1719,14 +1776,14 @@
     std::vector<uint64_t> ts((size_t)B * 48);
     for (int b = 0; b < 2 * B; b++) put_xyzz(Xyzz::inf(), &ts[24 * (size_t)b]);
     if (R) {
+        gb.ctl_cleared = false;
         accumulate_group(wk, gb, gp, gl, nullptr, table, s, R, (double)R * 128.0 / g.W);
         const uint64_t *res = reduce_group(gb, gp, gl, s, true);
         uint32_t exc = 0, nredo = 0;
         PNP_HIP(hipMemcpyAsync(ts.data(), res, ts.size() * 8, hipMemcpyDeviceToHost, s));
-        PNP_HIP(hipMemcpyAsync(&exc, gb.exc.p, 4, hipMemcpyDeviceToHost, s));
-        PNP_HIP(hipMemcpyAsync(&nredo, gb.redo.p, 4, hipMemcpyDeviceToHost, s));
-        wctr_fetch(gb, s);
+        ctl_fetch(gb, s);
         PNP_HIP(hipStreamSynchronize(s));
+        exc = gb.ctl_h.exc, nredo = gb.ctl_h.nredo;
         wctr_credit(wk, gb);
         if (wk.timer) wk.timer->credit("msm_redo_lanes", (double)nredo);
         if (exc) {
@@ -1767,7 +1824,7 @@
     uint64_t b = wk.digits.bytes + wk.part_counts.bytes + wk.rec_counts.bytes;
     for (const MsmGroup &g : wk.grp)
         b += g.counts.bytes + g.offsets.bytes + g.scan_tmp.bytes + g.ent.bytes + g.fkey.bytes + g.sorted.bytes +
-             g.buckets.bytes + g.seg.bytes + g.redo.bytes + g.exc.bytes + g.heavy.bytes + g.wctr.bytes;
+             g.buckets.bytes + g.seg.bytes + g.redo.bytes + g.ctl.bytes + g.heavy.bytes;
     return b;
 }
 
diff --git a/zprize23-gpu-submission_amd/csrc/msm_internal.h b/zprize23-gpu-submission_amd/csrc/msm_internal.h
--- a/zprize23-gpu-submission_amd/csrc/msm_internal.h
+++ b/zprize23-gpu-submission_amd/csrc/msm_internal.h
@@ -44,8 +44,8 @@
 #endif
 }
 void msm_merge_pieces29(const uint32_t *offs, uint64_t U, uint32_t S, uint64_t nthr, const uint32_t *tailb,
-                        const uint32_t *tlist, uint32_t *bk29, const uint32_t *head, const uint32_t *tail, uint32_t *exc,
-                        uint32_t *heavy, hipStream_t s);
+                        const uint32_t *ntail, const uint32_t *tlist, uint32_t *bk29, const uint32_t *head,
+                        const uint32_t *tail, uint32_t *exc, uint32_t *nheavy, uint32_t *heavy, hipStream_t s);
 void msm_merge_pieces29_exact(const uint32_t *offs, uint64_t U, uint32_t S, uint64_t nthr, uint32_t pieces,
                               const uint32_t *bk29, const uint32_t *head, const uint32_t *tail, uint64_t *bk,
                               hipStream_t s);
@@ -54,6 +54,6 @@
 const uint64_t *msm_reduce(const uint64_t *bk, uint64_t nwin, int NB, uint64_t *scratch,
                            hipStream_t s);
 const uint64_t *msm_reduce29(const uint32_t *bk29, const uint32_t *offs, uint64_t nwin, int NB,
-                             uint32_t *scratch, uint32_t *exc, hipStream_t s);
+                             uint32_t *scratch, uint32_t *exc, hipStream_t s, uint64_t *roots_out = nullptr);
 
 }
diff --git a/zprize23-gpu-submission_amd/csrc/msm_reduce.hip b/zprize23-gpu-submission_amd/csrc/msm_reduce.hip
--- a/zprize23-gpu-submission_amd/csrc/msm_reduce.hip
+++ b/zprize23-gpu-submission_amd/csrc/msm_reduce.hip
@@ -101,13 +101,14 @@
 #endif
 constexpr uint32_t MERGE_HEAVY = PNP_MERGE_HEAVY;
 __global__ __launch_bounds__(256) void k_merge_tails29(const uint32_t *offs, uint64_t U, uint64_t nthr, uint32_t S,
-                                                       const uint32_t *tailb, const uint32_t *tlist, uint32_t *bk29,
+                                                       const uint32_t *tailb, const uint32_t *ntail,
+                                                       const uint32_t *tlist, uint32_t *bk29,
                                                        const uint32_t *head, const uint32_t *tail, uint32_t *exc,
                                                        uint32_t *heavy, uint32_t *nheavy) {
     const uint64_t q = blockIdx.x * (uint64_t)blockDim.x + threadIdx.x;
-    if (q >= tlist[0]) return;
+    if (q >= *ntail) return;
     S = acc_seg(offs, U, nthr, S);
-    const uint64_t t = tlist[1 + q];
+    const uint64_t t = tlist[q];
     const uint32_t u = tailb[t];
     const uint32_t t1 = (offs[u + 1] - 1) / S;
     if (t1 - (uint32_t)t >= MERGE_HEAVY) {
@@ -148,14 +149,12 @@
 }
 
 void msm_merge_pieces29(const uint32_t *offs, uint64_t U, uint32_t S, uint64_t nthr, const uint32_t *tailb,
-                        const uint32_t *tlist, uint32_t *bk29, const uint32_t *head, const uint32_t *tail,
-                        uint32_t *exc, uint32_t *heavy, hipStream_t s) {
-    uint32_t *nheavy = heavy, *list = heavy + 1;
-    PNP_HIP(hipMemsetAsync(nheavy, 0, 4, s));
+                        const uint32_t *ntail, const uint32_t *tlist, uint32_t *bk29, const uint32_t *head,
+                        const uint32_t *tail, uint32_t *exc, uint32_t *nheavy, uint32_t *heavy, hipStream_t s) {
     hipLaunchKernelGGL(k_merge_tails29, dim3((uint32_t)((nthr + 255) / 256)), dim3(256), 0, s, offs, U, nthr, S,
-                       tailb, tlist, bk29, head, tail, exc, list, nheavy);
-    PNP_HIP(hipGetLastError());
-    hipLaunchKernelGGL(k_merge_heavy29, dim3(256), dim3(256), 0, s, offs, U, nthr, S, bk29, head, tail, exc, list,
+                       tailb, ntail, tlist, bk29, head, tail, exc, heavy, nheavy);
+    PNP_HIP(hipGetLastError());
+    hipLaunchKernelGGL(k_merge_heavy29, dim3(256), dim3(256), 0, s, offs, U, nthr, S, bk29, head, tail, exc, heavy,
                        nheavy);
     PNP_HIP(hipGetLastError());
 }
@@ -394,7 +393,7 @@
 }
 
 const uint64_t *msm_reduce29(const uint32_t *bk29, const uint32_t *offs, uint64_t nwin, int NB,
-                             uint32_t *scratch, uint32_t *exc, hipStream_t s) {
+                             uint32_t *scratch, uint32_t *exc, hipStream_t s, uint64_t *roots_out) {
 #ifndef PNP_LEAF_SMALL4
 #define PNP_LEAF_SMALL4 1
 #endif
@@ -405,7 +404,7 @@
     }
     uint64_t m = nwin * (uint64_t)NB / LW;
     uint32_t *a = scratch, *b = scratch + 168 * m;
-    uint64_t *roots = reinterpret_cast<uint64_t *>(scratch + 252 * m);
+    uint64_t *roots = roots_out ? roots_out : reinterpret_cast<uint64_t *>(scratch + 252 * m);
     const dim3 lgrid((uint32_t)((m + 255) / 256));
     static const uint64_t leaf_wide = [] {
         const char *e = getenv("PNP_LEAF_WIDE");
diff --git a/zprize23-gpu-submission_amd/csrc/pnp_internal.h b/zprize23-gpu-submission_amd/csrc/pnp_internal.h
--- a/zprize23-gpu-submission_amd/csrc/pnp_internal.h
+++ b/zprize23-gpu-submission_amd/csrc/pnp_internal.h
@@ -1,5 +1,6 @@
 #pragma once
 #include <hip/hip_runtime.h>
+#include <stddef.h>
 #include <stdint.h>
 #include <stdio.h>
 #include <map>
@@ -99,15 +100,25 @@
 extern thread_local bool t_bg_build;
 void bg_step(hipStream_t s);
 
+constexpr int WCTR_SLOTS = 64;
+struct MsmCtl {
+    uint32_t ntail, nredo, exc, nheavy;
+    uint32_t pad[12];
+    unsigned long long wctr[1 + WCTR_SLOTS];
+    unsigned long long pad2[7];
+};
+static_assert(offsetof(MsmCtl, wctr) == 64 && sizeof(MsmCtl) % 64 == 0, "MsmCtl: flags line, then the counters");
 struct MsmGroup {
     DevBuf counts, offsets, scan_tmp, ent, fkey, sorted, buckets, seg, redo;
-    DevBuf exc;
+    DevBuf ctl;
     DevBuf heavy;
     uint32_t S = 0, pieces = 0;
     uint64_t nthr = 0;
-    DevBuf wctr;
-    unsigned long long wctr_h[65] = {};
+    uint64_t WB = 0;
+    MsmCtl ctl_h = {};
     bool wctr_live = false;
+    bool ctl_cleared = false;
+    MsmCtl *ctl_dev() { return static_cast<MsmCtl *>(ctl.p); }
 };
 struct MsmWork {
     DevBuf digits;
@@ -157,6 +168,7 @@
 uint64_t msm_table_build_bytes(uint64_t n_points);
 uint64_t msm_work_bytes(uint64_t n_pts, uint64_t n_cfg, int fold_c, int B, uint64_t v_bytes, int world);
 uint64_t msm_work_held(const MsmWork &wk);
+void msm_work_recount(MsmWork &wk, hipStream_t s, unsigned long long ref[2], unsigned long long dev[2]);
 void msm_point_range(uint64_t n, int rank, int world, uint64_t &p0, uint64_t &p1);
 void msm_build_table(DevBuf &tab, const uint64_t *d_points, uint64_t n, int c, hipStream_t s);
 void xyzz_to_affine_dev(const uint64_t *xyzz, uint64_t n, uint64_t *aff, hipStream_t s);
diff --git a/zprize23-gpu-submission_amd/csrc/protocol.h b/zprize23-gpu-submission_amd/csrc/protocol.h
--- a/zprize23-gpu-submission_amd/csrc/protocol.h
+++ b/zprize23-gpu-submission_amd/csrc/protocol.h
@@ -70,9 +70,9 @@
                  const uint64_t *h1, const uint64_t *h2, const Fr &delta, const Fr &eps, uint64_t n,
                  hipStream_t s);
 void k_mul_inplace(uint64_t *a, const uint64_t *b, uint64_t n, hipStream_t s);
-bool k_any_nonzero(const uint64_t *v, uint64_t words, DevBuf &scratch, hipStream_t s);
+bool k_any_nonzero(const uint64_t *v, uint64_t words, DevBuf &scratch, hipStream_t s, unsigned *cleared = nullptr);
 void k_any_nonzero_n(const uint64_t *v, uint64_t words, uint64_t stride, int cnt, bool *nz, DevBuf &scratch,
-                     hipStream_t s);
+                     hipStream_t s, unsigned *cleared = nullptr);
 bool k_any_diff(const uint64_t *a, const uint64_t *b, uint64_t words, DevBuf &scratch, hipStream_t s);
 void k_hash_words(const uint64_t *a, uint64_t words, DevBuf &scratch, hipStream_t s, uint64_t out[2]);
 bool k_pack_affine(const uint8_t *src, uint64_t n, uint64_t stride, uint64_t x_off, uint64_t y_off,
@@ -83,6 +83,9 @@
 void k_widgets(const WidgetArgs &g, uint64_t N8, uint64_t *out, hipStream_t s);
 bool combine_split(pnp_ctx *ctx, const uint64_t *t, const uint64_t *f, uint64_t n, uint64_t *h1,
                    uint64_t *h2, hipStream_t s);
-void k_proof_marker(hipStream_t s);
+constexpr int PROOF_CTL_WORDS = 16;
+enum ProofCtl { PCTL_T_NZ = 0 , PCTL_TABLE_NZ = 2, PCTL_F_NZ = 3,
+                PCTL_WIRE_FLAG = 4, PCTL_Z_FLAG = 5  };
+void k_proof_marker(unsigned *ctl, hipStream_t s);
 
 }
diff --git a/zprize23-gpu-submission_amd/csrc/protocol.hip b/zprize23-gpu-submission_amd/csrc/protocol.hip
--- a/zprize23-gpu-submission_amd/csrc/protocol.hip
+++ b/zprize23-gpu-submission_amd/csrc/protocol.hip
@@ -124,10 +124,13 @@
     if (__any(acc != 0) && (threadIdx.x & 63) == 0) atomicOr(flag + blockIdx.y, 1u);
 }
 void k_any_nonzero_n(const uint64_t *v, uint64_t words, uint64_t stride, int cnt, bool *nz, DevBuf &scratch,
-                     hipStream_t s) {
-    if (scratch.bytes < 4 * (size_t)cnt + 16) scratch.alloc(4 * (size_t)cnt + 16);
-    unsigned *flag = static_cast<unsigned *>(scratch.p);
-    PNP_HIP(hipMemsetAsync(flag, 0, 4 * (size_t)cnt, s));
+                     hipStream_t s, unsigned *cleared) {
+    unsigned *flag = cleared;
+    if (!flag) {
+        if (scratch.bytes < 4 * (size_t)cnt + 16) scratch.alloc(4 * (size_t)cnt + 16);
+        flag = static_cast<unsigned *>(scratch.p);
+        PNP_HIP(hipMemsetAsync(flag, 0, 4 * (size_t)cnt, s));
+    }
     if (words) {
         uint64_t blocks = (words / 2 + 255) / 256;
         if (blocks > 2048) blocks = 2048;
@@ -141,9 +144,9 @@
     PNP_HIP(hipStreamSynchronize(s));
     for (int k = 0; k < cnt; k++) nz[k] = h[k] != 0;
 }
-bool k_any_nonzero(const uint64_t *v, uint64_t words, DevBuf &scratch, hipStream_t s) {
+bool k_any_nonzero(const uint64_t *v, uint64_t words, DevBuf &scratch, hipStream_t s, unsigned *cleared) {
     bool nz = false;
-    if (words) k_any_nonzero_n(v, words, words, 1, &nz, scratch, s);
+    if (words) k_any_nonzero_n(v, words, words, 1, &nz, scratch, s, cleared);
     return nz;
 }
 
@@ -444,9 +447,9 @@
 }
 
 namespace pnp {
-__global__ void k_proof_begin() {}
-void k_proof_marker(hipStream_t s) {
-    hipLaunchKernelGGL(k_proof_begin, dim3(1), dim3(1), 0, s);
-    PNP_HIP(hipGetLastError());
-}
-}
+__global__ void k_proof_begin(unsigned *ctl) { ctl[threadIdx.x] = 0; }
+void k_proof_marker(unsigned *ctl, hipStream_t s) {
+    hipLaunchKernelGGL(k_proof_begin, dim3(1), dim3(PROOF_CTL_WORDS), 0, s, ctl);
+    PNP_HIP(hipGetLastError());
+}
+}
diff --git a/zprize23-gpu-submission_amd/csrc/prover.cpp b/zprize23-gpu-submission_amd/csrc/prover.cpp
--- a/zprize23-gpu-submission_amd/csrc/prover.cpp
+++ b/zprize23-gpu-submission_amd/csrc/prover.cpp
@@ -158,7 +158,9 @@
     Timer tm(ctx);
     auto &nt = ctx->ntt;
     auto alg = [&](double elems) { ctx->ktimer.credit("proof_alg_bytes", 32.0 * elems); };
-    k_proof_marker(s);
+    unsigned *pctl = reinterpret_cast<unsigned *>(ctx->buf("proof_ctl", PROOF_CTL_WORDS * 4 / 32));
+    k_proof_marker(pctl, s);
+    ctx->proof_ctl = pctl;
     ntt_warm(nt, lg, s);
     const int world = ctx->msm.world;
     if (ctx->pk_blk_world != world || ctx->pk_blk_rank != ctx->msm.rank) {
@@ -274,11 +276,11 @@
     tr.append_scalar("zeta", zeta);
     uint64_t *tc = ctx->buf("tc", n), *table_poly = ctx->buf("table_poly", n);
     k_compress4(tc, pk.table1, pk.table2, pk.table3, pk.table4, zeta, n, s);
-    const bool table_zero = !k_any_nonzero(tc, 4 * n, ctx->scratch_b, s);
+    const bool table_zero = !k_any_nonzero(tc, 4 * n, ctx->scratch_b, s, pctl + PCTL_TABLE_NZ);
     uint64_t *fc = ctx->buf("fc", n), *f_poly = ctx->buf("f_poly", n);
     const uint64_t *wconst[4] = {wsc[0], wsc[1], wsc[2], wsc[3]};
     k_query_f(fc, qlk, qlk_rows, wconst, tc, zeta, n, s);
-    const bool f_zero = !k_any_nonzero(fc, 4 * n, ctx->scratch_b, s);
+    const bool f_zero = !k_any_nonzero(fc, 4 * n, ctx->scratch_b, s, pctl + PCTL_F_NZ);
     alg(5.0 * n + n + ng + n + n);
     if (!table_zero) ntt_run(nt, table_poly, lg, true, false, s, tc);
     if (!f_zero) ntt_run(nt, f_poly, lg, true, false, s, fc);
@@ -296,9 +298,6 @@
             oc[nc++] = &out->f_comm;
         }
         if (h_zero) {
-            PNP_HIP(hipMemsetAsync(h1, 0, 32 * n, s));
-            PNP_HIP(hipMemsetAsync(h2, 0, 32 * n, s));
-            alg(2.0 * n);
             set_infinity(&out->h_1_comm);
             set_infinity(&out->h_2_comm);
         } else {
@@ -378,12 +377,18 @@
     uint64_t *z2_poly = ctx->buf("z2_poly", n);
     const bool z2_one = h_zero;
     if (z2_one) {
-        uint64_t one[4];
-        to_u64_limbs(Fr::one(), one);
-        PNP_HIP(hipMemsetAsync(z2_poly, 0, 32 * n, s));
-        PNP_HIP(hipMemcpyAsync(z2_poly, one, 32, hipMemcpyHostToDevice, s));
-        PNP_HIP(hipStreamSynchronize(s));
+        if (ctx->z2_one_at != z2_poly || ctx->z2_one_n != n) {
+            uint64_t one[4];
+            to_u64_limbs(Fr::one(), one);
+            ctx->z2_one_at = nullptr;
+            PNP_HIP(hipMemsetAsync(z2_poly, 0, 32 * n, s));
+            PNP_HIP(hipMemcpyAsync(z2_poly, one, 32, hipMemcpyHostToDevice, s));
+            PNP_HIP(hipStreamSynchronize(s));
+            ctx->z2_one_at = z2_poly;
+            ctx->z2_one_n = n;
+        }
     } else {
+        ctx->z2_one_at = nullptr;
         if (lag && overlap) PNP_HIP(hipStreamWaitEvent(s, ctx->ev_z8, 0));
         k_lookup_nd(num, den, fc, tc, h1, h2, delta, eps, n, s);
         k_batch_inverse(den, n, ctx->scratch_a, s);
@@ -420,7 +425,7 @@
     tm.mark("r3_z2_pi");
 
     const Transcript tr3 = tr;
-    for (;;) {
+    for (int attempt = 0;; attempt++) {
         const uint64_t NBq = (uint64_t)nbq * n;
         Fr alpha = tr.challenge_scalar("alpha");
         tr.append_scalar("alpha", alpha);
@@ -603,8 +608,7 @@
         alg(2.0 * NBq + 2.0 * NBq);
         uint64_t *t_poly = ctx->buf("t_poly", 8 * len);
         const int npieces = dist ? 8 : nbq;
-        unsigned *t_nz = reinterpret_cast<unsigned *>(ctx->buf("t_nz", 1));
-        PNP_HIP(hipMemsetAsync(t_nz, 0, 4, s));
+        unsigned *t_nz = pctl + PCTL_T_NZ + attempt;
         if (!dist) {
             t_combine_blocks(nt, t_blk, nbq, t_poly, lg, t_nz, s);
         } else {
@@ -630,6 +634,8 @@
             }
             t_combine(nt, a2a + 4 * (uint64_t)nb * len * world, len, q0, t_poly, lg, t_nz, s);
         }
+        unsigned t_bits = 0;
+        PNP_HIP(hipMemcpyAsync(&t_bits, t_nz, 4, hipMemcpyDeviceToHost, s));
         tm.mark("r4_intt8");
         CommitmentC *tcm[8] = {&out->t_1_comm, &out->t_2_comm, &out->t_3_comm, &out->t_4_comm,
                                &out->t_5_comm, &out->t_6_comm, &out->t_7_comm, &out->t_8_comm};
@@ -638,12 +644,7 @@
             CommitmentC *oc[9];
             int nc = 0;
             uint64_t nz[8];
-            {
-                unsigned bits = 0;
-                PNP_HIP(hipMemcpyAsync(&bits, t_nz, 4, hipMemcpyDeviceToHost, s));
-                PNP_HIP(hipStreamSynchronize(s));
-                for (int k = 0; k < 8; k++) nz[k] = k < npieces && ((bits >> k) & 1);
-            }
+            for (int k = 0; k < 8; k++) nz[k] = k < npieces && ((t_bits >> k) & 1);
             if (dist) {
                 std::vector<uint64_t> all = shard_allgather(ctx, nz, 8, PNP_EX_TAG_T_FLAGS);
                 for (int k = 0; k < 8; k++) {
@@ -660,11 +661,8 @@
                 oc[nc++] = tcm[k];
             }
             if (z2_one) {
-                uint64_t g0[12];
-                PNP_HIP(hipMemcpyAsync(g0, ctx->ck_dev, sizeof g0, hipMemcpyDeviceToHost, s));
-                PNP_HIP(hipStreamSynchronize(s));
-                memcpy(out->z_2_comm.x, g0, 48);
-                memcpy(out->z_2_comm.y, g0 + 6, 48);
+                memcpy(out->z_2_comm.x, ctx->ck_g0, 48);
+                memcpy(out->z_2_comm.y, ctx->ck_g0 + 6, 48);
             } else if (dist) {
                 commit_affine(ctx, z2_poly, n, &out->z_2_comm);
             } else {
diff --git a/zprize23-gpu-submission_amd/csrc/wires.hip b/zprize23-gpu-submission_amd/csrc/wires.hip
--- a/zprize23-gpu-submission_amd/csrc/wires.hip
+++ b/zprize23-gpu-submission_amd/csrc/wires.hip
@@ -470,8 +470,7 @@
         return false;
     auto &wb = ctx->wb;
     hipStream_t s = ctx->stream;
-    uint32_t *flag = static_cast<uint32_t *>(wb.flag.p);
-    PNP_HIP(hipMemsetAsync(flag, 0, 4, s));
+    uint32_t *flag = ctx->proof_ctl + PCTL_WIRE_FLAG;
     WirePtrs wp{};
     for (int j = 0; j < 4; j++) {
         wp.w[j] = d_evals[j];
@@ -516,8 +515,7 @@
         return false;
     auto &wb = ctx->wb;
     hipStream_t s = ctx->stream;
-    uint32_t *flag = static_cast<uint32_t *>(wb.flag.p);
-    PNP_HIP(hipMemsetAsync(flag, 0, 4, s));
+    uint32_t *flag = ctx->proof_ctl + PCTL_Z_FLAG;
     WirePtrs wp{};
     wp.w[0] = d_z;
     wp.grp[0] = static_cast<const uint32_t *>(wb.grp[4].p);
diff --git a/zprize23-gpu-submission_amd/pnp/__init__.py b/zprize23-gpu-submission_amd/pnp/__init__.py
--- a/zprize23-gpu-submission_amd/pnp/__init__.py
+++ b/zprize23-gpu-submission_amd/pnp/__init__.py
@@ -24,7 +24,8 @@
            "pnp_set_exchange_v", "pnp_commit_segments", "pnp_hbm_usage",
            "pnp_ctx_stream", "pnp_set_exchange_ordered", "pnp_v1_context",
            "pnp_preprocess", "pnp_wire_sigma",
-           "pnp_load_wire_map", "pnp_gather_witness", "pnp_prove_assignment")
+           "pnp_load_wire_map", "pnp_gather_witness", "pnp_prove_assignment",
+           "pnp_msm_work_counters")
 
 
 ALLGATHER_FN = C.CFUNCTYPE(C.c_int, C.c_void_p, C.c_uint64)
@@ -83,6 +84,8 @@
     lib.pnp_set_exchange_ordered.argtypes = [vp, i32]
     lib.pnp_commit_segments.argtypes = [vp, vp, u64, i32, C.POINTER(u64), C.POINTER(vp), u64,
                                         C.POINTER(abi.CommitmentC)]
+    if hasattr(lib, "pnp_msm_work_counters"):
+        lib.pnp_msm_work_counters.argtypes = [vp, C.POINTER(u64), C.POINTER(u64)]
     lib.pnp_poly_eval.argtypes = [vp, vp, u64, vp, vp]
     lib.pnp_poly_div_linear.argtypes = [vp, vp, u64, vp]
     lib.pnp_prefix_product.argtypes = [vp, vp, u64]
@@ -97,6 +100,8 @@
     lib.pnp_load_commit_key_strided.argtypes = [vp, vp, u64, C.POINTER(abi.AffineLayout), i32]
     lib.pnp_proof_infinity_mask.argtypes = [C.POINTER(abi.ProofC)]
     for name in SYMBOLS:
+        if name == "pnp_msm_work_counters" and not hasattr(lib, name):
+            continue
         if name.startswith("pnp_") and name not in ("pnp_last_error", "pnp_ctx_destroy", "pnp_v1_context"):
             getattr(lib, name).restype = C.c_int if name != "pnp_last_error" else C.c_char_p
     lib.pnp_proof_infinity_mask.restype = C.c_uint32
@@ -294,6 +299,11 @@
               "pnp_commit_segments")
         return list(out)
 
+    def msm_work_counters(self):
+        ref, dev = (C.c_uint64 * 2)(), (C.c_uint64 * 2)()
+        check(self.lib.pnp_msm_work_counters(self.h, ref, dev), "pnp_msm_work_counters")
+        return (int(ref[0]), int(ref[1])), (int(dev[0]), int(dev[1]))
+
     def gather_witness(self, var, n_gates: int, values: int, n_vars: int, lg_n: int, w):
         V = (C.c_void_p * 4)(*[a or None for a in var])
         W = (C.c_void_p * 4)(*[a or None for a in w])
```

After: 0.1238 (median of 3 runs). Within noise of the previous version (-0.1%).
